# shehryar-malik/icrl

Hardware: AMD Instinct MI355X
Metric: env-steps/sec (ICRL outer loop, HCWithPos-v0) (higher is better)
Workload: dtype f32

## Files before the change

icrl_amd/csrc/ppo_common.h:

```cpp
#pragma once
#include "common.h"

namespace icrl {

typedef float f32x4 __attribute__((ext_vector_type(4)));
typedef unsigned long long u64;
#define MFMA_F32(a, b, c) __builtin_amdgcn_mfma_f32_16x16x4f32((a), (b), (c), 0, 0, 0)

constexpr int RB = 64;
constexpr int HD = 64;
constexpr int SH = 72;
constexpr int MAXB = 256;

struct TrainArgs {
  PolLayout L;
  float* params;
  float* exp_avg;
  float* exp_avg_sq;
  int* adam_t;
  icrl_buffer_t buf;
  const int* perms;
  const float* nu;
  icrl_ppo_hyper_t hp;
  float* stats;
  u64* xch;
  unsigned t_magic;
  const struct PlanStep* plan_steps;
  const struct PlanChunk* plan_chunks;
  int n_steps;
  u64* gx;
};

struct PlanStep {
  float step_size, inv_bc2_sqrt;
  int nb_flags;

  int perm_base;
};
constexpr int NB_MASK = 0x3ff, NB_FIRST = 10, NB_LAST = 11, NB_EPOCH = 12;
struct PlanChunk {
  int perm_base, rows;
};

__device__ __forceinline__ float sum16(float v) { return row_sum(v); }

__device__ __forceinline__ float tile_colsum(const f32x4& t) {
  return quad_rows_sum((t[0] + t[1]) + (t[2] + t[3]));
}

__device__ __forceinline__ unsigned long long stamp() {
  unsigned long long t;
  asm volatile("s_memtime %0\n\ts_waitcnt lgkmcnt(0)" : "=s"(t)::"memory");
  return t;
}
#define STAMP(slot)                                                        \
  if (prof) {                                                              \
    __builtin_amdgcn_sched_barrier(0);                                     \
    const unsigned long long now_ = stamp();                               \
    __builtin_amdgcn_sched_barrier(0);                                     \
    ph[slot] += now_ - t_last;                                             \
    t_last = now_;                                                         \
  }

__device__ __forceinline__ void lds_barrier() { asm volatile("s_waitcnt lgkmcnt(0)\n\ts_barrier" ::: "memory"); }

__device__ __forceinline__ f32x4 lds128(const float* p) { return *reinterpret_cast<const f32x4*>(p); }

__device__ __forceinline__ void acc_put(float& slot, float v) { asm("v_accvgpr_write_b32 %0, %1" : "=a"(slot) : "v"(v)); }
__device__ __forceinline__ void acc_set(float& slot, float v) { asm("v_accvgpr_write_b32 %0, %1" : "+a"(slot) : "v"(v)); }
__device__ __forceinline__ float acc_get(const float& slot) {
  float v;
  asm("v_accvgpr_read_b32 %0, %1" : "=v"(v) : "a"(slot));
  return v;
}

struct Cursor {
  int e, p, m;
};

constexpr int XCD_STRIDE = 8;
__device__ __forceinline__ int xcc_word(int j) { return j < 4 ? 28 + j : 56 + j; }
__device__ __forceinline__ int xcc_word12(int j) { return j < 8 ? 24 + j : 48 + j; }
__device__ __forceinline__ bool run_on_one_xcd(unsigned long long* xch, int j, int M, bool wide = false) {
  const unsigned long long me = 0x100ull | (unsigned long long)xcc_id();
  __hip_atomic_store(xch + (wide ? xcc_word12(j) : xcc_word(j)), me, __ATOMIC_RELAXED, __HIP_MEMORY_SCOPE_AGENT);
  bool same = true;
  for (int o = 0; o < M; ++o) {
    if (o == j) continue;
    unsigned long long v = 0;
    for (int spins = 0; spins < (1 << 18); ++spins) {
      v = __hip_atomic_load(xch + (wide ? xcc_word12(o) : xcc_word(o)), __ATOMIC_RELAXED, __HIP_MEMORY_SCOPE_AGENT);
      if (v != 0) break;
      __builtin_amdgcn_s_sleep(8);
    }
    same = same && v == me;
  }
  return same;
}
__device__ __forceinline__ bool packed_slot(int M, int n_runs, int& run, int& j) {
  const int id = (int)blockIdx.x, per = XCD_STRIDE * M;
  run = (id / per) * XCD_STRIDE + (id & (XCD_STRIDE - 1));
  j = (id % per) / XCD_STRIDE;
  return run < n_runs;
}
inline int packed_grid(int M, int n_runs) {
  static const bool off = getenv("ICRL_NO_XCD_PACK") != nullptr;
  static const int cus_per_xcd = [] {
    int dev = 0, cus = 0;
    if (hipGetDevice(&dev) != hipSuccess || hipDeviceGetAttribute(&cus, hipDeviceAttributeMultiprocessorCount, dev) != hipSuccess || cus < XCD_STRIDE) return 32;
    return cus / XCD_STRIDE;
  }();
  const int groups = (n_runs + XCD_STRIDE - 1) / XCD_STRIDE;
  if (off || groups * M > cus_per_xcd - 2) return 0;
  return n_runs >= XCD_STRIDE ? groups * XCD_STRIDE * M : XCD_STRIDE * (M - 1) + n_runs;
}
template <class K>
inline int launch_update_single(K kernel, int M, dim3 block, size_t dyn_lds, hipStream_t s, TrainArgs& arg) {
  const int pg = packed_grid(M, 1);
  hipError_t e = launch_coresident(kernel, dim3(pg ? pg : M), block, dyn_lds, s, arg, pg ? 1 : 0);
  if (e == hipErrorCooperativeLaunchTooLarge && pg) {
    (void)hipGetLastError();
    e = launch_coresident(kernel, dim3(M), block, dyn_lds, s, arg, 0);
  }
  return (int)e;
}

#if defined(__HIP_DEVICE_COMPILE__) && !defined(__gfx950__) && !defined(__gfx942__)
#error "libicrl_hip: the XCD-local exchange of the persistent kernels is written for gfx950 (CDNA4) / gfx942"
#endif

int launch_train_rows(const TrainArgs& a, int nt1, bool discrete, bool split, hipStream_t s);
int launch_train_pairs(const TrainArgs& a, int nt1, bool discrete, hipStream_t s);
int launch_train_halves(const TrainArgs& a, bool discrete, int parts, hipStream_t s);
int launch_train_halves_batch(const TrainArgs* d_args, int n_runs, int obs, bool discrete, int parts, bool prof, hipStream_t s);
int launch_train_quarters_wide(const TrainArgs& a, bool discrete, hipStream_t s);
int launch_train_quarters_wide2(const TrainArgs& a, bool discrete, hipStream_t s);
constexpr int HALVES_MAX_RUNS = 40;
constexpr int QUARTERS_MAX_RUNS = 16;
int launch_train_rows_batch(const TrainArgs* d_args, int n_runs, int nt1, bool discrete, bool split, hipStream_t s);
int launch_train_pairs_batch(const TrainArgs* d_args, int n_runs, int obs, int nt1, bool discrete, bool prof, hipStream_t s);


}
```

icrl_amd/csrc/ppo_train.hip:

```cpp
#include "ppo_common.h"

namespace icrl {

constexpr int TH = 512;
constexpr int SO = 24;

template <int NT1>
struct Smem {
  static constexpr int O16 = 16 * NT1, SX = O16 + 8;
  static constexpr int W1 = 0;
  static constexpr int W2 = W1 + HD * SX;
  static constexpr int WH = W2 + HD * SH;
  static constexpr int B1 = WH + 16 * SH;
  static constexpr int B2 = B1 + HD;
  static constexpr int BH = B2 + HD;
  static constexpr int LS = BH + 16;
  static constexpr int X = LS + 16;
  static constexpr int H1 = X + RB * SX;
  static constexpr int H2 = H1 + RB * SH;
  static constexpr int DZ = H2 + RB * SH;
  static constexpr int DO = DZ + RB * SH;
  static constexpr int RED1 = DO + RB * SO;
  static constexpr int RED2 = RED1 + 4 * HD;
  static constexpr int PBH = RED2 + 4 * HD;
  static constexpr int PLS = PBH + 64;
  static constexpr int PST = PLS + 64;
  static constexpr int MISC = PST + 32;
  static constexpr int GAU = MISC + 48;
  static constexpr int TOTAL = GAU + 48;
  static constexpr int ACT = DZ, OLP = DZ + 16, ADR = DZ + 17, ADC = DZ + 18;
};

template <int NT1, bool DISC>
__global__ void __launch_bounds__(TH, 2) ppo_train_kernel(TrainArgs a) {
  using S = Smem<NT1>;
  constexpr int SX = S::SX;
  constexpr int NT1H = NT1 / 2;
  constexpr int XR = (SX + 7) / 8;
  static_assert(NT1 >= 2, "obs tiles are split between the two column halves");
  extern __shared__ __attribute__((aligned(16))) float sm[];
  const int role = blockIdx.x;
  const int tid = threadIdx.x;
  const int lane = tid & 63;
  const int w = __builtin_amdgcn_readfirstlane(tid >> 6);
  const int rt = w & 3, hf = w >> 2;
  const int r = lane & 15, q = lane >> 4;
  const PolLayout& L = a.L;
  const int O = L.O, A = L.A;
  const int n_out = role == 0 ? A : 1;
  const int T = a.buf.T, N = a.buf.N;
  const int n_total = T * N;
  const int B = a.hp.batch_size;
  const int n_mb = (n_total + B - 1) / B;
  const int n_epochs = a.hp.n_epochs;
  const float nu = a.nu[0];

  const int gW1 = L.W1[role], gb1 = L.b1[role], gW2 = L.W2[role], gb2 = L.b2[role];
  const int gWh = role == 0 ? L.Wa : (role == 1 ? L.Wv : L.Wc);
  const int gbh = role == 0 ? L.ba : (role == 1 ? L.bv : L.bc);

  for (int i = tid; i < HD * SX; i += TH) { const int j = i / SX, k = i % SX; sm[S::W1 + i] = k < O ? a.params[gW1 + j * O + k] : 0.f; }
  for (int i = tid; i < HD * SH; i += TH) { const int j = i / SH, k = i % SH; sm[S::W2 + i] = k < HD ? a.params[gW2 + j * HD + k] : 0.f; }
  for (int i = tid; i < 16 * SH; i += TH) { const int o = i / SH, k = i % SH; sm[S::WH + i] = (o < n_out && k < HD) ? a.params[gWh + o * HD + k] : 0.f; }
  if (tid < HD) { sm[S::B1 + tid] = a.params[gb1 + tid]; sm[S::B2 + tid] = a.params[gb2 + tid]; }
  if (tid < 16) { sm[S::BH + tid] = tid < n_out ? a.params[gbh + tid] : 0.f; sm[S::LS + tid] = (!DISC && role == 0 && tid < A) ? a.params[L.log_std + tid] : 0.f; }

  f32x4 mW1[NT1H], vW1[NT1H], gW1r[NT1H], mW2[2], vW2[2], gW2r[2], mWh, vWh, gWhr;
#pragma unroll
  for (int c = 0; c < NT1H; ++c)
#pragma unroll
    for (int i = 0; i < 4; ++i) {
      const int j = 16 * rt + 4 * q + i, k = 16 * (hf * NT1H + c) + r;
      mW1[c][i] = k < O ? a.exp_avg[gW1 + j * O + k] : 0.f;
      vW1[c][i] = k < O ? a.exp_avg_sq[gW1 + j * O + k] : 0.f;
    }
#pragma unroll
  for (int c = 0; c < 2; ++c)
#pragma unroll
    for (int i = 0; i < 4; ++i) {
      const int j = 16 * rt + 4 * q + i, k = 16 * (2 * hf + c) + r;
      mW2[c][i] = a.exp_avg[gW2 + j * HD + k];
      vW2[c][i] = a.exp_avg_sq[gW2 + j * HD + k];
    }
#pragma unroll
  for (int i = 0; i < 4; ++i) {
    const int o = 4 * q + i, j = 16 * rt + r;
    const bool own = hf == 0 && o < n_out;
    mWh[i] = own ? a.exp_avg[gWh + o * HD + j] : 0.f;
    vWh[i] = own ? a.exp_avg_sq[gWh + o * HD + j] : 0.f;
  }
  int vec_g = -1, vec_s = 0;
  if (tid < 64) { vec_g = gb1 + tid; vec_s = S::B1 + tid; }
  else if (tid < 128) { vec_g = gb2 + tid - 64; vec_s = S::B2 + tid - 64; }
  else if (tid < 144) { if (tid - 128 < n_out) { vec_g = gbh + tid - 128; vec_s = S::BH + tid - 128; } }
  else if (tid < 160) { if (!DISC && role == 0 && tid - 144 < A) { vec_g = L.log_std + tid - 144; vec_s = S::LS + tid - 144; } }
  float mB = 0.f, vB = 0.f, gB = 0.f;
  if (vec_g >= 0) { mB = a.exp_avg[vec_g]; vB = a.exp_avg_sq[vec_g]; }

  const int t0 = a.adam_t[0];
  double b1pow = pow((double)a.hp.adam_beta1, (double)t0), b2pow = pow((double)a.hp.adam_beta2, (double)t0);
  const float w1 = (float)(1.0 - (double)a.hp.adam_beta1);
  const float w2 = (float)(1.0 - (double)a.hp.adam_beta2);
  const float clip = a.hp.clip_range;
  const float vclip = role == 1 ? a.hp.clip_range_reward_vf : a.hp.clip_range_cost_vf;
  const float vcoef = role == 1 ? a.hp.reward_vf_coef : a.hp.cost_vf_coef;

  auto cur_rows = [&](const Cursor& c) {
    int left = B - c.m;
    if (n_total - c.p < left) left = n_total - c.p;
    return left < RB ? left : RB;
  };
  auto cur_advance = [&](Cursor c) {
    const int rows = cur_rows(c);
    c.p += rows; c.m += rows;
    if (c.p >= n_total) { c.p = 0; c.m = 0; ++c.e; }
    else if (c.m >= B) c.m = 0;
    return c;
  };
  auto to_off = [&](int idx) -> unsigned {
    unsigned env = __umulhi((unsigned)idx, a.t_magic);
    int t = idx - (int)env * T;
    if (t >= T) { t -= T; ++env; }
    if (t >= T) { t -= T; ++env; }
    return (unsigned)t * (unsigned)N + env;
  };
  const int gb_row = tid >> 3, gpart = tid & 7;
  auto load_idx = [&](const Cursor& c) -> int {
    if (c.e >= n_epochs || gb_row >= cur_rows(c)) return -1;
    return a.perms[(size_t)c.e * n_total + c.p + gb_row];
  };
  float px[XR], pact[2], psc0 = 0.f, psc1 = 0.f, psc2 = 0.f;
  auto issue_rows = [&](int idx) {
    const bool valid = idx >= 0;
    const size_t off = valid ? (size_t)to_off(idx) : 0;
    const float* orow = a.buf.observations + off * O;
#pragma unroll
    for (int i = 0; i < XR; ++i) { const int k = gpart + 8 * i; px[i] = (valid && k < O) ? orow[k] : 0.f; }
    if (role == 0) {
      const float* arow = a.buf.actions + off * a.buf.act_store;
#pragma unroll
      for (int i = 0; i < 2; ++i) { const int k = gpart + 8 * i; pact[i] = (valid && k < a.buf.act_store) ? arow[k] : 0.f; }
      if (gpart == 0) {
        psc0 = valid ? a.buf.log_probs[off] : 0.f;
        psc1 = valid ? a.buf.reward_advantages[off] : 0.f;
        psc2 = valid ? a.buf.cost_advantages[off] : 0.f;
      }
    } else if (gpart == 0) {
      const float* rets = role == 1 ? a.buf.reward_returns : a.buf.cost_returns;
      const float* olds = role == 1 ? a.buf.reward_values : a.buf.cost_values;
      psc1 = valid ? rets[off] : 0.f;
      psc0 = valid ? olds[off] : 0.f;
    }
  };
  auto commit_rows = [&]() {
#pragma unroll
    for (int i = 0; i < XR; ++i) { const int k = gpart + 8 * i; if (k < SX) sm[S::X + gb_row * SX + k] = px[i]; }
    if (role == 0) {
#pragma unroll
      for (int i = 0; i < 2; ++i) sm[S::ACT + gb_row * SH + gpart + 8 * i] = pact[i];
      if (gpart == 0) { sm[S::OLP + gb_row * SH] = psc0; sm[S::ADR + gb_row * SH] = psc1; sm[S::ADC + gb_row * SH] = psc2; }
    } else if (gpart == 0) {
      sm[S::OLP + gb_row * SH] = psc0; sm[S::ADR + gb_row * SH] = psc1;
    }
  };
  float sar = 0.f, sac = 0.f;
  auto mb_rows_at = [&](int p) { const int left = n_total - p; return left < B ? left : B; };
  auto stat_idx = [&](int e, int p) -> int {
    if (role != 0 || e >= n_epochs || tid >= mb_rows_at(p)) return -1;
    return a.perms[(size_t)e * n_total + p + tid];
  };
  auto issue_stats = [&](int idx) {
    sar = 0.f; sac = 0.f;
    if (idx >= 0) {
      const unsigned off = to_off(idx);
      sar = a.buf.reward_advantages[off];
      sac = a.buf.cost_advantages[off];
    }
  };
  float mean_r = 0.f, std_r = 1.f, mean_c = 0.f;
  auto compute_stats = [&](int nb) {
    if (role != 0) return;
    const bool in = tid < nb;
    float s_r = wave_sum_fast(in ? sar : 0.f), s_c = wave_sum_fast(in ? sac : 0.f), s_rr = wave_sum_fast(in ? sar * sar : 0.f);
    lds_barrier();
    if (lane == 0) { sm[S::MISC + 16 + w] = s_r; sm[S::MISC + 24 + w] = s_c; sm[S::MISC + 32 + w] = s_rr; }
    lds_barrier();
    s_r = sm[S::MISC + 16] + sm[S::MISC + 17];
    s_c = sm[S::MISC + 24] + sm[S::MISC + 25];
    s_rr = sm[S::MISC + 32] + sm[S::MISC + 33];
    mean_r = s_r / (float)nb;
    mean_c = s_c / (float)nb;
    const float var = fmaxf(s_rr - s_r * mean_r, 0.f) / (float)(nb - 1);
    std_r = sqrtf(var);
  };
  auto refresh_gauss = [&]() {
    if (!DISC && role == 0 && tid >= 144 && tid < 160) {
      const int k = tid - 144;
      const float sd = __expf(sm[S::LS + k]);
      const float iv = __builtin_amdgcn_rcpf(sd * sd);
      sm[S::GAU + k] = k < A ? iv : 0.f;
      sm[S::GAU + 16 + k] = k < A ? 0.5f * iv : 0.f;
      sm[S::GAU + 32 + k] = k < A ? __logf(sd) + LOG_SQRT_2PI_F : 0.f;
    }
  };
  float st_ent = 0.f, st_pg = 0.f, st_vl = 0.f, st_cf = 0.f, last_loss = 0.f;
  int steps_done = 0, early_stop_epoch = n_epochs, status = 0;
  if (tid == 0) { sm[S::MISC + 12] = 0.f; sm[S::MISC + 13] = 0.f; }

  Cursor c_nx2 = cur_advance(Cursor{0, 0, 0});
  int idx_next = load_idx(c_nx2);
  c_nx2 = cur_advance(c_nx2);
  int idx_nx2 = load_idx(c_nx2);
  issue_rows(load_idx(Cursor{0, 0, 0}));
  issue_stats(stat_idx(0, 0));
  refresh_gauss();
  int s_e = 0, s_p = mb_rows_at(0);
  if (s_p >= n_total) { s_p = 0; s_e = 1; }
  int sidx_next = stat_idx(s_e, s_p);
  __syncthreads();
  commit_rows();
  compute_stats(mb_rows_at(0));
  __syncthreads();

  const bool prof = (a.hp._pad & 1) != 0;
  unsigned long long ph[8] = {0, 0, 0, 0, 0, 0, 0, 0};
  unsigned long long t_last = prof ? stamp() : 0ull;

  unsigned step = 0;
  bool stop = false;
  for (int epoch = 0; epoch < n_epochs && !stop; ++epoch) {
    float kl_sum = 0.f;
    for (int mb = 0; mb < n_mb && !stop; ++mb) {
      ++step;
      const int nb = mb_rows_at(mb * B);
      const float c_mean_r = mean_r, c_mean_c = mean_c;
      const float c_istd_r = 1.f / (std_r + 1e-8f);
      const float cpol_nb = 1.f / ((1.f + nu) * (float)nb);
      issue_stats(sidx_next);
      {
        s_p += mb_rows_at(s_p);
        if (s_p >= n_total) { s_p = 0; ++s_e; }
        sidx_next = stat_idx(s_e, s_p);
      }
#pragma unroll
      for (int c = 0; c < NT1H; ++c) gW1r[c] = f32x4{0.f, 0.f, 0.f, 0.f};
#pragma unroll
      for (int c = 0; c < 2; ++c) gW2r[c] = f32x4{0.f, 0.f, 0.f, 0.f};
      gWhr = f32x4{0.f, 0.f, 0.f, 0.f};
      gB = 0.f;
      float mb_s0 = 0.f, mb_s1 = 0.f, mb_s2 = 0.f, mb_s3 = 0.f, mb_s4 = 0.f;

      const int n_chunks = (nb + RB - 1) / RB;
      for (int ch = 0; ch < n_chunks; ++ch) {
        const int nrows = (nb - ch * RB) < RB ? (nb - ch * RB) : RB;
        if (ch > 0) {
          commit_rows();
          lds_barrier();
        }
        f32x4 h1t[2], h2t[2];
        {
          f32x4 av[NT1], bv[2][NT1];
          const float* pa = sm + S::X + (16 * rt + r) * SX + 4 * q;
          const float* pb = sm + S::W1 + (32 * hf + r) * SX + 4 * q;
#pragma unroll
          for (int js = 0; js < NT1; ++js) {
            av[js] = lds128(pa + 16 * js);
#pragma unroll
            for (int c = 0; c < 2; ++c) bv[c][js] = lds128(pb + c * 16 * SX + 16 * js);
          }
          __builtin_amdgcn_sched_barrier(0);
          f32x4 acc[2];
#pragma unroll
          for (int c = 0; c < 2; ++c) acc[c] = f32x4{0.f, 0.f, 0.f, 0.f};
#pragma unroll
          for (int js = 0; js < NT1; ++js)
#pragma unroll
            for (int e = 0; e < 4; ++e)
#pragma unroll
              for (int c = 0; c < 2; ++c) acc[c] = MFMA_F32(av[js][e], bv[c][js][e], acc[c]);
#pragma unroll
          for (int c = 0; c < 2; ++c) {
            const int col = 32 * hf + 16 * c + r;
            const float bias = sm[S::B1 + col];
#pragma unroll
            for (int i = 0; i < 4; ++i) {
              h1t[c][i] = fast_tanh(acc[c][i] + bias);
              sm[S::H1 + (16 * rt + 4 * q + i) * SH + col] = h1t[c][i];
            }
          }
        }
        issue_rows(idx_next);
        idx_next = idx_nx2;
        c_nx2 = cur_advance(c_nx2);
        idx_nx2 = load_idx(c_nx2);
        lds_barrier();
        {
          f32x4 av[4], bv[2][4];
          const float* pa = sm + S::H1 + (16 * rt + r) * SH + 4 * q;
          const float* pb = sm + S::W2 + (32 * hf + r) * SH + 4 * q;
#pragma unroll
          for (int js = 0; js < 4; ++js) {
            av[js] = lds128(pa + 16 * js);
#pragma unroll
            for (int c = 0; c < 2; ++c) bv[c][js] = lds128(pb + c * 16 * SH + 16 * js);
          }
          __builtin_amdgcn_sched_barrier(0);
          f32x4 acc[2];
#pragma unroll
          for (int c = 0; c < 2; ++c) acc[c] = f32x4{0.f, 0.f, 0.f, 0.f};
#pragma unroll
          for (int js = 0; js < 4; ++js)
#pragma unroll
            for (int e = 0; e < 4; ++e)
#pragma unroll
              for (int c = 0; c < 2; ++c) acc[c] = MFMA_F32(av[js][e], bv[c][js][e], acc[c]);
#pragma unroll
          for (int c = 0; c < 2; ++c) {
            const int col = 32 * hf + 16 * c + r;
            const float bias = sm[S::B2 + col];
#pragma unroll
            for (int i = 0; i < 4; ++i) {
              h2t[c][i] = fast_tanh(acc[c][i] + bias);
              sm[S::H2 + (16 * rt + 4 * q + i) * SH + col] = h2t[c][i];
            }
          }
        }
        lds_barrier();
        if (hf == 0) {
          f32x4 av[4], bv[4];
          const float* pa = sm + S::H2 + (16 * rt + r) * SH + 4 * q;
          const float* pb = sm + S::WH + r * SH + 4 * q;
#pragma unroll
          for (int js = 0; js < 4; ++js) { av[js] = lds128(pa + 16 * js); bv[js] = lds128(pb + 16 * js); }
          __builtin_amdgcn_sched_barrier(0);
          f32x4 acc[4];
#pragma unroll
          for (int js = 0; js < 4; ++js) {
            acc[js] = f32x4{0.f, 0.f, 0.f, 0.f};
#pragma unroll
            for (int e = 0; e < 4; ++e) acc[js] = MFMA_F32(av[js][e], bv[js][e], acc[js]);
          }
          const float bias = sm[S::BH + r];
#pragma unroll
          for (int i = 0; i < 4; ++i)
            sm[S::DO + (16 * rt + 4 * q + i) * SO + r] = ((acc[0][i] + acc[1][i]) + (acc[2][i] + acc[3][i])) + bias;
        }
        lds_barrier();
        STAMP(0)
        {
          const int b = 16 * rt + r;
          const bool valid = b < nrows;
          float* dor = sm + S::DO + b * SO;
          if (role == 0 && DISC) {
            float lg[4], pr[4], zmax = -INFINITY;
#pragma unroll
            for (int i = 0; i < 4; ++i) {
              const int k = q + 4 * i;
              lg[i] = k < A ? dor[k] : -INFINITY;
              zmax = fmaxf(zmax, lg[i]);
            }
            zmax = xor16_max(xor32_max(zmax));
            float se = 0.f;
#pragma unroll
            for (int i = 0; i < 4; ++i) se += (q + 4 * i < A) ? expf(lg[i] - zmax) : 0.f;
            se = quad_rows_sum(se);
            const float lse = zmax + logf(se);
            const int act = (int)sm[S::ACT + b * SH];
            float lp = 0.f, ent = 0.f;
#pragma unroll
            for (int i = 0; i < 4; ++i) {
              const int k = q + 4 * i;
              lg[i] = k < A ? lg[i] - lse : 0.f;
              pr[i] = k < A ? expf(lg[i]) : 0.f;
              lp += (k == act) ? lg[i] : 0.f;
              ent -= pr[i] * lg[i];
            }
            lp = quad_rows_sum(lp);
            ent = quad_rows_sum(ent);
            const float old_lp = sm[S::OLP + b * SH];
            const float ratio = __expf(lp - old_lp);
            const float Ar = (sm[S::ADR + b * SH] - c_mean_r) * c_istd_r;
            const float Ac = sm[S::ADC + b * SH] - c_mean_c;
            const float s1 = Ar * ratio;
            const float rc = fminf(fmaxf(ratio, 1.f - clip), 1.f + clip);
            const float s2 = Ar * rc;
            const float gsel = (s1 <= s2) ? Ar : 0.f;
            const float dlp = valid ? cpol_nb * (-gsel + nu * Ac) * ratio : 0.f;
            const float dent = valid ? a.hp.ent_coef / (float)nb : 0.f;
            lds_barrier();
#pragma unroll
            for (int ii = 0; ii < 2; ++ii) {
              const int k = q + 4 * (2 * hf + ii);
              const float pk = hf == 0 ? pr[ii] : pr[2 + ii];
              const float lk = hf == 0 ? lg[ii] : lg[2 + ii];
              const float dk = k < A ? dlp * ((k == act ? 1.f : 0.f) - pk) + dent * (pk * (lk + ent)) : 0.f;
              dor[k] = dk;
              const float colsum = sum16(dk);
              if (r == 0) { sm[S::PBH + rt * 16 + k] = colsum; sm[S::PLS + rt * 16 + k] = 0.f; }
            }
            if (hf == 0) {
              const float v0 = sum16(valid ? fminf(s1, s2) : 0.f);
              const float v1 = sum16(valid ? Ac * ratio : 0.f);
              const float v2 = sum16(valid ? (fabsf(ratio - 1.f) > clip ? 1.f : 0.f) : 0.f);
              const float v3 = sum16(valid ? old_lp - lp : 0.f);
              const float v4 = sum16(valid ? ent : 0.f);
              if (lane == 0) { sm[S::PST + rt * 8 + 0] = v0; sm[S::PST + rt * 8 + 1] = v1; sm[S::PST + rt * 8 + 2] = v2; sm[S::PST + rt * 8 + 3] = v3; sm[S::PST + rt * 8 + 4] = v4; }
            }
          } else if (role == 0) {
            float dd[4], iv[4];
            float lp = 0.f;
#pragma unroll
            for (int i = 0; i < 4; ++i) {
              const int k = q + 4 * i;
              dd[i] = sm[S::ACT + b * SH + k] - dor[k];
              iv[i] = sm[S::GAU + k];
              lp += -(dd[i] * dd[i]) * sm[S::GAU + 16 + k] - sm[S::GAU + 32 + k];
            }
            lp = quad_rows_sum(lp);
            const float old_lp = sm[S::OLP + b * SH];
            const float ratio = __expf(lp - old_lp);
            const float Ar = (sm[S::ADR + b * SH] - c_mean_r) * c_istd_r;
            const float Ac = sm[S::ADC + b * SH] - c_mean_c;
            const float s1 = Ar * ratio;
            const float rc = fminf(fmaxf(ratio, 1.f - clip), 1.f + clip);
            const float s2 = Ar * rc;
            const float gsel = (s1 <= s2) ? Ar : 0.f;
            const float dlp = valid ? cpol_nb * (-gsel + nu * Ac) * ratio : 0.f;
            lds_barrier();
#pragma unroll
            for (int ii = 0; ii < 2; ++ii) {
              const int i = 2 * hf + ii;
              const int k = q + 4 * i;
              const float ddi = hf == 0 ? dd[ii] : dd[2 + ii];
              const float ivi = hf == 0 ? iv[ii] : iv[2 + ii];
              const float dk = dlp * (ddi * ivi);
              const float lk = (k < A) ? dlp * ((ddi * ddi) * ivi - 1.f) : 0.f;
              dor[k] = dk;
              const float colsum = sum16(dk);
              const float lssum = sum16(lk);
              if (r == 0) { sm[S::PBH + rt * 16 + k] = colsum; sm[S::PLS + rt * 16 + k] = lssum; }
            }
            if (hf == 0) {
              const float v0 = sum16(valid ? fminf(s1, s2) : 0.f);
              const float v1 = sum16(valid ? Ac * ratio : 0.f);
              const float v2 = sum16(valid ? (fabsf(ratio - 1.f) > clip ? 1.f : 0.f) : 0.f);
              const float v3 = sum16(valid ? old_lp - lp : 0.f);
              if (lane == 0) { sm[S::PST + rt * 8 + 0] = v0; sm[S::PST + rt * 8 + 1] = v1; sm[S::PST + rt * 8 + 2] = v2; sm[S::PST + rt * 8 + 3] = v3; }
            }
          } else {
            const float v = dor[0];
            const float R = sm[S::ADR + b * SH];
            float vp = v, pass = 1.f;
            if (vclip >= 0.f) {
              const float old = sm[S::OLP + b * SH];
              const float dv = v - old;
              vp = old + fminf(fmaxf(dv, -vclip), vclip);
              pass = (dv >= -vclip && dv <= vclip) ? 1.f : 0.f;
            }
            const float e = vp - R;
            const float d0 = valid ? vcoef * 2.f * e / (float)nb * pass : 0.f;
            lds_barrier();
            if (hf == 0) {
              if (q == 0) {
                dor[0] = d0;
#pragma unroll
                for (int k = 1; k < 16; ++k) dor[k] = 0.f;
              }
              const float colsum = sum16(d0);
              const float se = sum16(valid ? e * e : 0.f);
              if (lane == 0) {
                sm[S::PBH + rt * 16] = colsum;
#pragma unroll
                for (int k = 1; k < 16; ++k) sm[S::PBH + rt * 16 + k] = 0.f;
                sm[S::PST + rt * 8 + 0] = se;
              }
            }
          }
        }
        lds_barrier();
        STAMP(1)
        {
          const f32x4 av = lds128(sm + S::DO + (16 * rt + r) * SO + 4 * q);
          float bv[2][4];
          const float* pb = sm + S::WH + (4 * q) * SH + 32 * hf + r;
#pragma unroll
          for (int e = 0; e < 4; ++e)
#pragma unroll
            for (int c = 0; c < 2; ++c) bv[c][e] = pb[e * SH + 16 * c];
          f32x4 acc[2];
#pragma unroll
          for (int c = 0; c < 2; ++c) acc[c] = f32x4{0.f, 0.f, 0.f, 0.f};
#pragma unroll
          for (int e = 0; e < 4; ++e)
#pragma unroll
            for (int c = 0; c < 2; ++c) acc[c] = MFMA_F32(av[e], bv[c][e], acc[c]);
#pragma unroll
          for (int c = 0; c < 2; ++c) {
            const int col = 32 * hf + 16 * c + r;
#pragma unroll
            for (int i = 0; i < 4; ++i) {
              acc[c][i] = acc[c][i] * (1.f - h2t[c][i] * h2t[c][i]);
              sm[S::DZ + (16 * rt + 4 * q + i) * SH + col] = acc[c][i];
            }
            const float cs = tile_colsum(acc[c]);
            if (q == 0) sm[S::RED2 + rt * HD + col] = cs;
          }
        }
        lds_barrier();
        if (hf == 0) {
          float av[4][4], bv[4][4];
          const float* pa = sm + S::DO + (4 * q) * SO + r;
          const float* pb = sm + S::H2 + (4 * q) * SH + 16 * rt + r;
#pragma unroll
          for (int js = 0; js < 4; ++js)
#pragma unroll
            for (int e = 0; e < 4; ++e) { av[js][e] = pa[(16 * js + e) * SO]; bv[js][e] = pb[(16 * js + e) * SH]; }
          __builtin_amdgcn_sched_barrier(0);
          f32x4 acc[4];
#pragma unroll
          for (int js = 0; js < 4; ++js) {
            acc[js] = f32x4{0.f, 0.f, 0.f, 0.f};
#pragma unroll
            for (int e = 0; e < 4; ++e) acc[js] = MFMA_F32(av[js][e], bv[js][e], acc[js]);
          }
#pragma unroll
          for (int i = 0; i < 4; ++i) gWhr[i] += (acc[0][i] + acc[1][i]) + (acc[2][i] + acc[3][i]);
        }
        if (tid >= 64 && tid < 128) {
          const int j = tid - 64;
          gB += (sm[S::RED2 + j] + sm[S::RED2 + HD + j]) + (sm[S::RED2 + 2 * HD + j] + sm[S::RED2 + 3 * HD + j]);
        } else if (tid >= 128 && tid < 144) {
          const int k = tid - 128;
          gB += (sm[S::PBH + k] + sm[S::PBH + 16 + k]) + (sm[S::PBH + 32 + k] + sm[S::PBH + 48 + k]);
        } else if (tid >= 144 && tid < 160) {
          const int k = tid - 144;
          gB += (sm[S::PLS + k] + sm[S::PLS + 16 + k]) + (sm[S::PLS + 32 + k] + sm[S::PLS + 48 + k]);
        }
        if (tid == 0) {
          mb_s0 += (sm[S::PST + 0] + sm[S::PST + 8]) + (sm[S::PST + 16] + sm[S::PST + 24]);
          mb_s1 += (sm[S::PST + 1] + sm[S::PST + 9]) + (sm[S::PST + 17] + sm[S::PST + 25]);
          mb_s2 += (sm[S::PST + 2] + sm[S::PST + 10]) + (sm[S::PST + 18] + sm[S::PST + 26]);
          mb_s3 += (sm[S::PST + 3] + sm[S::PST + 11]) + (sm[S::PST + 19] + sm[S::PST + 27]);
          if (DISC) mb_s4 += (sm[S::PST + 4] + sm[S::PST + 12]) + (sm[S::PST + 20] + sm[S::PST + 28]);
        }
        lds_barrier();
        {
          f32x4 av[4];
          const float* pa = sm + S::DZ + (16 * rt + r) * SH + 4 * q;
          const float* pb = sm + S::W2 + (4 * q) * SH + 32 * hf + r;
#pragma unroll
          for (int js = 0; js < 4; ++js) av[js] = lds128(pa + 16 * js);
          float bv[4][2][4];
#pragma unroll
          for (int js = 0; js < 4; ++js)
#pragma unroll
            for (int e = 0; e < 4; ++e)
#pragma unroll
              for (int c = 0; c < 2; ++c) bv[js][c][e] = pb[(16 * js + e) * SH + 16 * c];
          __builtin_amdgcn_sched_barrier(0);
          f32x4 acc[2];
#pragma unroll
          for (int c = 0; c < 2; ++c) acc[c] = f32x4{0.f, 0.f, 0.f, 0.f};
#pragma unroll
          for (int js = 0; js < 4; ++js)
#pragma unroll
            for (int e = 0; e < 4; ++e)
#pragma unroll
              for (int c = 0; c < 2; ++c) acc[c] = MFMA_F32(av[js][e], bv[js][c][e], acc[c]);
          float a2[4][4], b2v[4][2][4];
          const float* pa2 = sm + S::DZ + (4 * q) * SH + 16 * rt + r;
          const float* pb2 = sm + S::H1 + (4 * q) * SH + 32 * hf + r;
#pragma unroll
          for (int js = 0; js < 4; ++js)
#pragma unroll
            for (int e = 0; e < 4; ++e) {
              a2[js][e] = pa2[(16 * js + e) * SH];
#pragma unroll
              for (int c = 0; c < 2; ++c) b2v[js][c][e] = pb2[(16 * js + e) * SH + 16 * c];
            }
#pragma unroll
          for (int js = 0; js < 4; ++js)
#pragma unroll
            for (int e = 0; e < 4; ++e)
#pragma unroll
              for (int c = 0; c < 2; ++c) gW2r[c] = MFMA_F32(a2[js][e], b2v[js][c][e], gW2r[c]);
#pragma unroll
          for (int c = 0; c < 2; ++c) {
            const int col = 32 * hf + 16 * c + r;
#pragma unroll
            for (int i = 0; i < 4; ++i) {
              acc[c][i] = acc[c][i] * (1.f - h1t[c][i] * h1t[c][i]);
              sm[S::H2 + (16 * rt + 4 * q + i) * SH + col] = acc[c][i];
            }
            const float cs = tile_colsum(acc[c]);
            if (q == 0) sm[S::RED1 + rt * HD + col] = cs;
          }
        }
        lds_barrier();
        {
          float av[4][4];
          const float* pa = sm + S::H2 + (4 * q) * SH + 16 * rt + r;
          const float* pb = sm + S::X + (4 * q) * SX + 16 * hf * NT1H + r;
#pragma unroll
          for (int js = 0; js < 4; ++js)
#pragma unroll
            for (int e = 0; e < 4; ++e) av[js][e] = pa[(16 * js + e) * SH];
#pragma unroll
          for (int js = 0; js < 4; ++js) {
            float bv[NT1H][4];
#pragma unroll
            for (int e = 0; e < 4; ++e)
#pragma unroll
              for (int c = 0; c < NT1H; ++c) bv[c][e] = pb[(16 * js + e) * SX + 16 * c];
#pragma unroll
            for (int e = 0; e < 4; ++e)
#pragma unroll
              for (int c = 0; c < NT1H; ++c) gW1r[c] = MFMA_F32(av[js][e], bv[c][e], gW1r[c]);
          }
        }
        if (tid < 64) gB += (sm[S::RED1 + tid] + sm[S::RED1 + HD + tid]) + (sm[S::RED1 + 2 * HD + tid] + sm[S::RED1 + 3 * HD + tid]);
        lds_barrier();
        STAMP(2)
      }

      if (!DISC && role == 0 && tid >= 144 && tid < 144 + A) gB += -a.hp.ent_coef;

      float ss = 0.f;
#pragma unroll
      for (int c = 0; c < NT1H; ++c)
#pragma unroll
        for (int i = 0; i < 4; ++i) ss += gW1r[c][i] * gW1r[c][i];
#pragma unroll
      for (int c = 0; c < 2; ++c)
#pragma unroll
        for (int i = 0; i < 4; ++i) ss += gW2r[c][i] * gW2r[c][i];
#pragma unroll
      for (int i = 0; i < 4; ++i) ss += gWhr[i] * gWhr[i];
      if (vec_g >= 0) ss += gB * gB;
      ss = wave_sum_fast(ss);
      if (lane == 0) sm[S::MISC + w] = ss;
      lds_barrier();
      if (tid == 0) {
        ss = ((sm[S::MISC + 0] + sm[S::MISC + 1]) + (sm[S::MISC + 2] + sm[S::MISC + 3])) +
             ((sm[S::MISC + 4] + sm[S::MISC + 5]) + (sm[S::MISC + 6] + sm[S::MISC + 7]));
        bool want_stop = false;
        float mean_kl = 0.f;
        if (role == 0) {
          kl_sum += mb_s3 / (float)nb;
          if (mb == n_mb - 1) {
            mean_kl = kl_sum / (float)n_mb;
            if (a.hp.use_target_kl && mean_kl > 1.5f * a.hp.target_kl) { want_stop = true; early_stop_epoch = epoch; }
          }
        }
        const unsigned tag = step | (want_stop ? 0x80000000u : 0u);
        __hip_atomic_store(a.xch + (step & 1) * 4 + role, ((u64)tag << 32) | (u64)__float_as_uint(ss), __ATOMIC_RELAXED,
                           __HIP_MEMORY_SCOPE_AGENT);
        ++steps_done;
        if (role == 0) {
          float ent = 0.f;
          if (DISC) ent = mb_s4 / (float)nb;
          else for (int k = 0; k < A; ++k) ent += HALF_LOG_2PI_PLUS_HALF_F + sm[S::LS + k];
          const float entropy_loss = -ent;
          const float pl = (-(mb_s0 / (float)nb) + nu * (mb_s1 / (float)nb)) / (1.f + nu);
          st_ent += entropy_loss; st_pg += pl; st_cf += mb_s2 / (float)nb;
          last_loss = pl + a.hp.ent_coef * entropy_loss;
          if (mb == n_mb - 1) { a.stats[32 + epoch] = mean_kl; a.stats[7] = mean_kl; }
        } else {
          const float vl = mb_s0 / (float)nb;
          st_vl += vl;
          last_loss = vl;
        }
      }
      STAMP(3)
      commit_rows();
      {
        const int pn = (mb + 1 < n_mb) ? (mb + 1) * B : 0;
        compute_stats(mb_rows_at(pn));
      }
      STAMP(4)
      if (tid < 3) {
        u64 v = 0;
        int spins = 0;
        bool ok = false;
        while (spins < (1 << 24)) {
          v = __hip_atomic_load(a.xch + (step & 1) * 4 + tid, __ATOMIC_RELAXED, __HIP_MEMORY_SCOPE_AGENT);
          if ((unsigned)((v >> 32) & 0x7fffffffu) == step) { ok = true; break; }
          __builtin_amdgcn_s_sleep(1);
          ++spins;
        }
        sm[S::MISC + 8 + tid] = __uint_as_float((unsigned)(v & 0xffffffffu));
        if (tid == 0) sm[S::MISC + 12] = (v >> 63) ? 1.f : 0.f;
        if (!ok) sm[S::MISC + 13] = 1.f;
      } else if (tid == 3) {
        b1pow *= (double)a.hp.adam_beta1;
        b2pow *= (double)a.hp.adam_beta2;
        sm[S::MISC + 14] = (float)((double)a.hp.lr / (1.0 - b1pow));
        sm[S::MISC + 15] = (float)(1.0 / sqrt(1.0 - b2pow));
      }
      lds_barrier();
      STAMP(5)
      const float total = sqrtf((sm[S::MISC + 8] + sm[S::MISC + 9]) + sm[S::MISC + 10]);
      stop = sm[S::MISC + 12] != 0.f;
      if (sm[S::MISC + 13] != 0.f) { status = 1; stop = true; }
      float coef = a.hp.max_grad_norm / (total + 1e-6f);
      coef = coef > 1.f ? 1.f : coef;

      const float step_size = sm[S::MISC + 14];
      const float inv_bc2_sqrt = sm[S::MISC + 15];
      const float b2f = a.hp.adam_beta2, epsf = a.hp.adam_eps;
      auto adam = [&](float g, float& m, float& v, float p) -> float {
        g = g * coef;
        m = m + (g - m) * w1;
        v = v * b2f + w2 * (g * g);
        const float denom = __builtin_amdgcn_sqrtf(v) * inv_bc2_sqrt + epsf;
        return p - step_size * (m * __builtin_amdgcn_rcpf(denom));
      };
      if (status == 0) {
#pragma unroll
        for (int c = 0; c < NT1H; ++c)
#pragma unroll
          for (int i = 0; i < 4; ++i) {
            const int j = 16 * rt + 4 * q + i, k = 16 * (hf * NT1H + c) + r;
            if (k < O) { float* pw = sm + S::W1 + j * SX + k; float m_ = mW1[c][i], v_ = vW1[c][i]; *pw = adam(gW1r[c][i], m_, v_, *pw); mW1[c][i] = m_; vW1[c][i] = v_; }
          }
#pragma unroll
        for (int c = 0; c < 2; ++c)
#pragma unroll
          for (int i = 0; i < 4; ++i) {
            float* pw = sm + S::W2 + (16 * rt + 4 * q + i) * SH + 16 * (2 * hf + c) + r;
            float m_ = mW2[c][i], v_ = vW2[c][i];
            *pw = adam(gW2r[c][i], m_, v_, *pw);
            mW2[c][i] = m_; vW2[c][i] = v_;
          }
        if (hf == 0) {
#pragma unroll
          for (int i = 0; i < 4; ++i) {
            const int o = 4 * q + i;
            if (o < n_out) { float* pw = sm + S::WH + o * SH + 16 * rt + r; float m_ = mWh[i], v_ = vWh[i]; *pw = adam(gWhr[i], m_, v_, *pw); mWh[i] = m_; vWh[i] = v_; }
          }
        }
        if (vec_g >= 0) sm[vec_s] = adam(gB, mB, vB, sm[vec_s]);
        refresh_gauss();
      }
      if (tid == 0) { sm[S::MISC + 12] = 0.f; sm[S::MISC + 13] = 0.f; }
      lds_barrier();
      STAMP(6)
    }
  }

  __syncthreads();
  for (int i = tid; i < HD * O; i += TH) { const int j = i / O, k = i % O; a.params[gW1 + i] = sm[S::W1 + j * SX + k]; }
  for (int i = tid; i < HD * HD; i += TH) { const int j = i / HD, k = i % HD; a.params[gW2 + i] = sm[S::W2 + j * SH + k]; }
  for (int i = tid; i < n_out * HD; i += TH) { const int o = i / HD, k = i % HD; a.params[gWh + i] = sm[S::WH + o * SH + k]; }
  if (vec_g >= 0) { a.params[vec_g] = sm[vec_s]; a.exp_avg[vec_g] = mB; a.exp_avg_sq[vec_g] = vB; }
#pragma unroll
  for (int c = 0; c < NT1H; ++c)
#pragma unroll
    for (int i = 0; i < 4; ++i) {
      const int j = 16 * rt + 4 * q + i, k = 16 * (hf * NT1H + c) + r;
      if (k < O) { a.exp_avg[gW1 + j * O + k] = mW1[c][i]; a.exp_avg_sq[gW1 + j * O + k] = vW1[c][i]; }
    }
#pragma unroll
  for (int c = 0; c < 2; ++c)
#pragma unroll
    for (int i = 0; i < 4; ++i) {
      const int j = 16 * rt + 4 * q + i, k = 16 * (2 * hf + c) + r;
      a.exp_avg[gW2 + j * HD + k] = mW2[c][i];
      a.exp_avg_sq[gW2 + j * HD + k] = vW2[c][i];
    }
  if (hf == 0) {
#pragma unroll
    for (int i = 0; i < 4; ++i) {
      const int o = 4 * q + i, j = 16 * rt + r;
      if (o < n_out) { a.exp_avg[gWh + o * HD + j] = mWh[i]; a.exp_avg_sq[gWh + o * HD + j] = vWh[i]; }
    }
  }
  if (tid == 0 && prof) {
    for (int k = 0; k < 7; ++k) {
      const int slot = 12 + 7 * role + k;
      if (slot < 32) a.stats[slot] = (float)((double)ph[k] / (double)(steps_done > 0 ? steps_done : 1));
    }
  }
  if (tid == 0) {
    if (role == 0) {
      a.stats[0] = (float)early_stop_epoch;
      a.stats[1] = (float)steps_done;
      a.stats[2] = st_ent; a.stats[3] = st_pg; a.stats[6] = st_cf;
      a.stats[8] = last_loss;
      a.stats[11] = (float)status;
      a.adam_t[0] = t0 + steps_done;
    } else if (role == 1) {
      a.stats[4] = st_vl; a.stats[9] = last_loss;
    } else {
      a.stats[5] = st_vl; a.stats[10] = last_loss;
    }
  }
}

__global__ void ppo_perm_offsets_kernel(const int* __restrict__ perms, long long n, int T, int N, int* __restrict__ out) {
  const long long i = (long long)blockIdx.x * blockDim.x + threadIdx.x;
  if (i >= n) return;
  const int idx = perms[i];
  const int env = idx / T, t = idx - env * T;
  out[i] = t * N + env;
}

__global__ void ppo_plan_kernel(const int* adam_t, int n_steps, int n_mb, int n_total, int B, double lr, double b1, double b2,
                                PlanStep* steps, PlanChunk* chunks, int two_per_step) {
  const int i = blockIdx.x * blockDim.x + threadIdx.x;
  if (i >= n_steps + 2) return;
  if (i >= n_steps) { steps[i] = PlanStep{0.f, 0.f, 0, 0}; return; }
  const int e = i / n_mb, mb = i % n_mb, p = mb * B;
  const int nb = n_total - p < B ? n_total - p : B;
  const int cpm = (B + RB - 1) / RB;
  const int nb_last = n_total - (n_mb - 1) * B;
  const int cpe = (n_mb - 1) * cpm + (nb_last + RB - 1) / RB;
  const int g0 = e * cpe + mb * cpm, nch = (nb + RB - 1) / RB;
  const double t = (double)(adam_t[0] + i + 1);
  steps[i] = PlanStep{(float)(lr / (1.0 - pow(b1, t))), (float)(1.0 / sqrt(1.0 - pow(b2, t))),
                      nb | ((mb == 0) << NB_FIRST) | ((mb == n_mb - 1) << NB_LAST) | (e << NB_EPOCH), e * n_total + p};
  if (chunks == nullptr) return;
  if (two_per_step) {
    for (int c = 0; c < 2; ++c) chunks[2 * i + c] = c < nch ? PlanChunk{e * n_total + p + RB * c, nb - RB * c < RB ? nb - RB * c : RB} : PlanChunk{0, 0};
    if (i == n_steps - 1)
      for (int c = 0; c < 10; ++c) chunks[2 * n_steps + c] = PlanChunk{0, 0};
    return;
  }
  for (int c = 0; c < nch; ++c) chunks[g0 + c] = PlanChunk{e * n_total + p + RB * c, nb - RB * c < RB ? nb - RB * c : RB};
  if (i == n_steps - 1)
    for (int c = 0; c < 5; ++c) chunks[g0 + nch + c] = PlanChunk{0, 0};
}

}

using namespace icrl;

template <int NT1, bool DISC>
static int launch_train(const TrainArgs& a, hipStream_t s) {
  static_assert(Smem<NT1>::TOTAL * sizeof(float) <= 160 * 1024, "LDS budget");
  const size_t bytes = (size_t)Smem<NT1>::TOTAL * sizeof(float);
  hipError_t e = hipFuncSetAttribute((const void*)ppo_train_kernel<NT1, DISC>, hipFuncAttributeMaxDynamicSharedMemorySize, (int)bytes);
  if (e != hipSuccess) return (int)e;
  TrainArgs arg = a;
  return (int)launch_coresident(ppo_train_kernel<NT1, DISC>, dim3(3), dim3(TH), bytes, s, arg);
}

static bool quarters_default() {
  static const int v = [] { const char* e = getenv("ICRL_QUARTERS"); return e != nullptr ? (e[0] == '1' ? 1 : 0) : 1; }();
  return v != 0;
}

static int prepare_train(const icrl_policy_t* pol, float* exp_avg, float* exp_avg_sq, int32_t* adam_step, const icrl_buffer_t* buf,
                         const int32_t* perms, const float* nu, const icrl_ppo_hyper_t* hp, float* stats, void* sync_ws,
                         hipStream_t s, TrainArgs& a, int* err, int n_runs) {
  auto bad = [&](int e) { *err = e; return -1; };
  if (pol->arch != nullptr || pol->h1 != HD || pol->h2 != HD)
    return bad(fail("icrl_ppo_lag_train: hidden widths (%d, %d)%s; the persistent update kernels are built for %d x %d (the reference's default net_arch)", pol->h1, pol->h2,
                    pol->arch != nullptr ? " with an `arch` descriptor" : "", HD, HD));
  if (pol->obs_dim < 1 || pol->obs_dim > 128 || pol->act_dim < 1 || pol->act_dim > 16)
    return bad(fail("icrl_ppo_lag_train: obs_dim %d (1..128) / act_dim %d (1..16)", pol->obs_dim, pol->act_dim));
  if (hp->batch_size < 2 || hp->batch_size > MAXB || hp->n_epochs < 1)
    return bad(fail("icrl_ppo_lag_train: batch_size %d (2..%d: one minibatch = at most four 64-row chunks of one workgroup), n_epochs %d (>= 1)", hp->batch_size, MAXB, hp->n_epochs));
  if (hp->n_epochs >= (1 << 19)) return bad(fail("icrl_ppo_lag_train: n_epochs %d, limit 2^19", hp->n_epochs));
  if (hp->batch_size > 128 && (hp->_pad & 2))
    return bad(fail("icrl_ppo_lag_train: batch_size %d: the column-split tiles kernel (hp->_pad & 2) stops at 128 rows", hp->batch_size));
  if (buf->obs_dim != pol->obs_dim || buf->T < 1)
    return bad(fail("icrl_ppo_lag_train: buffer obs_dim %d vs policy %d, T = %d", buf->obs_dim, pol->obs_dim, buf->T));
  if ((long long)buf->T * buf->N >= (1ll << 31) || (long long)buf->T * buf->N * (pol->obs_dim > 16 ? pol->obs_dim : 16) >= (1ll << 30))
    return bad(fail("icrl_ppo_lag_train: %d x %d transitions x obs_dim %d overflow the kernel's 32-bit element offsets (limit 2^30 floats per plane)", buf->T, buf->N, pol->obs_dim));
  if (pol->discrete && buf->act_store != 1) return bad(fail("icrl_ppo_lag_train: discrete policy needs act_store = 1 (action index), got %d", buf->act_store));
  a.L = make_pol_layout(pol->obs_dim, pol->act_dim, pol->h1, pol->h2, pol->discrete);
  a.params = pol->params; a.exp_avg = exp_avg; a.exp_avg_sq = exp_avg_sq; a.adam_t = adam_step;
  a.buf = *buf; a.perms = perms; a.nu = nu; a.hp = *hp; a.stats = stats; a.xch = (u64*)sync_ws;
  a.t_magic = buf->T == 1 ? 0xFFFFFFFFu : (unsigned)((1ull << 32) / (unsigned long long)buf->T);
  a.plan_steps = nullptr; a.plan_chunks = nullptr; a.n_steps = 0; a.gx = nullptr;
  hipError_t e = hipMemsetAsync(sync_ws, 0, 512, s);
  if (e != hipSuccess) return bad((int)e);
  e = hipMemsetAsync(stats, 0, (32 + hp->n_epochs) * sizeof(float), s);
  if (e != hipSuccess) return bad((int)e);
  const int nt1 = (pol->obs_dim + 15) / 16;
  if (nt1 > 8 || (hp->_pad & 2)) {
    if (hp->batch_size > 128) return bad(fail("icrl_ppo_lag_train: batch_size %d with obs_dim %d: the column-split tiles kernel stops at 128 rows", hp->batch_size, pol->obs_dim));
    return 3;
  }
  const int n_total = buf->T * buf->N;
  const int n_mb = (n_total + hp->batch_size - 1) / hp->batch_size;
  const long long n_steps = (long long)hp->n_epochs * n_mb;
  if (n_steps >= (1ll << 21)) return bad(fail("icrl_ppo_lag_train: %lld optimiser steps per call, limit 2^21", n_steps));
  PlanStep* steps = reinterpret_cast<PlanStep*>((char*)sync_ws + 512);
  PlanChunk* chunks = reinterpret_cast<PlanChunk*>(steps + n_steps + 2);
  a.plan_steps = steps; a.plan_chunks = chunks; a.n_steps = (int)n_steps;
  {
    int* offs = reinterpret_cast<int*>((char*)sync_ws + ICRL_PPO_PLAN_BYTES(n_steps));
    const long long n = (long long)hp->n_epochs * n_total;
    hipLaunchKernelGGL(ppo_perm_offsets_kernel, dim3((unsigned)((n + 255) / 256)), dim3(256), 0, s, perms, n, buf->T, buf->N, offs);
    a.perms = offs;
  }
  const bool quarters_wide = nt1 > 4 && n_runs == 1 && !(hp->_pad & (4 | 32)) && quarters_default();
  static const bool one_pass = [] { const char* e = getenv("ICRL_QUARTERS_PASSES"); return e == nullptr || e[0] != '1'; }();
  const bool quarters_wide2 = quarters_wide && one_pass && hp->batch_size > RB && hp->batch_size <= 2 * RB;
  const bool rows = !quarters_wide && ((hp->_pad & 4) || nt1 > 4);
  const bool split = rows && hp->batch_size > RB && hp->batch_size <= 2 * RB && !(hp->_pad & 8);
  const bool halves = !rows && n_runs <= HALVES_MAX_RUNS && nt1 <= 2 && !(hp->_pad & 16);
  const bool quarters = halves && n_runs <= QUARTERS_MAX_RUNS && !(hp->_pad & 32) && quarters_default();
  hipLaunchKernelGGL(ppo_plan_kernel, dim3((unsigned)((n_steps + 2 + 255) / 256)), dim3(256), 0, s, adam_step, (int)n_steps, n_mb,
                     n_total, hp->batch_size, (double)hp->lr, (double)hp->adam_beta1, (double)hp->adam_beta2, steps, chunks, (int)(split || quarters_wide2));
  if (split || halves || quarters_wide) {
    const size_t off = (ICRL_PPO_PLAN_BYTES(n_steps) + 4 * (size_t)hp->n_epochs * n_total + 255) / 256 * 256;
    a.gx = reinterpret_cast<u64*>((char*)sync_ws + off);
    e = hipMemsetAsync(a.gx, 0, ICRL_PPO_SPLIT_BYTES, s);
    if (e != hipSuccess) return bad((int)e);
  }
  if (quarters_wide) return quarters_wide2 ? 7 : 6;
  return rows ? (split ? 2 : 1) : (halves ? (quarters ? 5 : 4) : 0);
}

static int train_generic(const icrl_policy_t* pol, float* exp_avg, float* exp_avg_sq, int32_t* adam_step, const icrl_buffer_t* buf,
                         const int32_t* perms, const float* nu, const icrl_ppo_hyper_t* hp, float* stats, void* sync_ws, hipStream_t s) {
  if (hp->batch_size < 2 || hp->n_epochs < 1) return fail("icrl_ppo_lag_train: batch_size %d (>= 2), n_epochs %d (>= 1)", hp->batch_size, hp->n_epochs);
  if (pol->arch != nullptr) { if (int e = policy_generic_check(pol, "icrl_ppo_lag_train")) return e; }
  else if (pol->h1 != pol->h2 || pol->h1 % 64 != 0 || pol->h1 > 256 || pol->obs_dim < 1 || pol->obs_dim > 1024 || pol->act_dim < 1 || pol->act_dim > 16)
    return fail("icrl_ppo_lag_train: hidden widths (%d, %d), obs_dim %d, act_dim %d: the persistent kernels are built for %d x %d (narrower layers stored "
                "zero-padded), obs <= 128, act <= 16; the generic-shape path for a common padded width that is a multiple of 64 up to 256, obs <= 1024",
                pol->h1, pol->h2, pol->obs_dim, pol->act_dim, HD, HD);
  if (buf->obs_dim != pol->obs_dim || buf->T < 1) return fail("icrl_ppo_lag_train: buffer obs_dim %d vs policy %d, T = %d", buf->obs_dim, pol->obs_dim, buf->T);
  if ((long long)buf->T * buf->N * (pol->obs_dim > 16 ? pol->obs_dim : 16) >= (1ll << 31))
    return fail("icrl_ppo_lag_train: %d x %d transitions x obs_dim %d overflow 32-bit element offsets", buf->T, buf->N, pol->obs_dim);
  if (pol->discrete && buf->act_store != 1) return fail("icrl_ppo_lag_train: discrete policy needs act_store = 1 (action index), got %d", buf->act_store);
  const int n_total = buf->T * buf->N;
  const int n_mb = (n_total + hp->batch_size - 1) / hp->batch_size;
  const long long n_steps = (long long)hp->n_epochs * n_mb;
  hipError_t e = hipMemsetAsync(stats, 0, (32 + hp->n_epochs) * sizeof(float), s);
  if (e != hipSuccess) return (int)e;
  int* offs = reinterpret_cast<int*>((char*)sync_ws + ICRL_PPO_PLAN_BYTES(n_steps));
  const long long n = (long long)hp->n_epochs * n_total;
  hipLaunchKernelGGL(ppo_perm_offsets_kernel, dim3((unsigned)((n + 255) / 256)), dim3(256), 0, s, perms, n, buf->T, buf->N, offs);
  char* scratch = (char*)sync_ws + ICRL_PPO_SYNC_BYTES(hp->n_epochs, n_mb, n_total);
  const int err = launch_train_generic(pol, exp_avg, exp_avg_sq, adam_step, buf, offs, nu, hp, stats, scratch, sync_ws, s);
  if (err == 0 && !policy_is_wide(pol)) return icrl_policy_prepare(pol, (void*)s);
  return err;
}

extern "C" int icrl_ppo_generic_row_floats(const icrl_policy_t* pol) { return generic_row_floats(pol); }

extern "C" int icrl_ppo_lag_train(const icrl_policy_t* pol, float* exp_avg, float* exp_avg_sq, int32_t* adam_step,
                                  const icrl_buffer_t* buf, const int32_t* perms, const float* nu,
                                  const icrl_ppo_hyper_t* hp, float* stats, void* sync_ws, void* stream) {
  TrainArgs a;
  hipStream_t s = (hipStream_t)stream;
  if (policy_is_wide(pol) || hp->batch_size > MAXB)
    return train_generic(pol, exp_avg, exp_avg_sq, adam_step, buf, perms, nu, hp, stats, sync_ws, s);
  int err = 0;
  const int kind = prepare_train(pol, exp_avg, exp_avg_sq, adam_step, buf, perms, nu, hp, stats, sync_ws, s, a, &err, 1);
  if (kind < 0) return err;
  const int nt1 = (pol->obs_dim + 15) / 16;
  if (kind == 4 || kind == 5) return launch_train_halves(a, pol->discrete != 0, kind == 5 ? 4 : 2, s);
  if (kind == 6) return launch_train_quarters_wide(a, pol->discrete != 0, s);
  if (kind == 7) return launch_train_quarters_wide2(a, pol->discrete != 0, s);
  if (kind == 0) return launch_train_pairs(a, nt1, pol->discrete != 0, s);
  if (kind <= 2) return launch_train_rows(a, nt1, pol->discrete != 0, kind == 2, s);
  if (pol->discrete) {
    if (nt1 <= 2) return launch_train<2, true>(a, s);
    if (nt1 <= 4) return launch_train<4, true>(a, s);
    return launch_train<8, true>(a, s);
  }
  if (nt1 <= 2) return launch_train<2, false>(a, s);
  if (nt1 <= 4) return launch_train<4, false>(a, s);
  return launch_train<8, false>(a, s);
}

extern "C" int icrl_ppo_lag_train_batch(int n_runs, const icrl_ppo_train_job_t* jobs, void* args_ws, long long args_ws_bytes,
                                        void* stream) {
  if (n_runs < 1 || n_runs > 65535) return fail("icrl_ppo_lag_train_batch: n_runs = %d (1..65535)", n_runs);
  if (args_ws == nullptr || args_ws_bytes < (long long)n_runs * (long long)sizeof(TrainArgs))
    return fail("icrl_ppo_lag_train_batch: args_ws holds %lld B, %d runs need %lld (ICRL_BATCH_ARGS_BYTES each)", args_ws_bytes, n_runs,
                (long long)n_runs * (long long)sizeof(TrainArgs));
  static_assert(sizeof(TrainArgs) <= ICRL_BATCH_ARGS_BYTES, "ICRL_BATCH_ARGS_BYTES");
  hipStream_t s = (hipStream_t)stream;
  TrainArgs* d_args = (TrainArgs*)args_ws;
  int kind0 = -1;
  const icrl_ppo_train_job_t& j0 = jobs[0];
  for (int r = 0; r < n_runs; ++r) {
    const icrl_ppo_train_job_t& j = jobs[r];
    if (j.pol->obs_dim != j0.pol->obs_dim || j.pol->act_dim != j0.pol->act_dim || j.pol->discrete != j0.pol->discrete ||
        j.hp->batch_size != j0.hp->batch_size || j.hp->n_epochs != j0.hp->n_epochs || j.hp->_pad != j0.hp->_pad ||
        j.buf->T != j0.buf->T || j.buf->N != j0.buf->N || j.buf->act_store != j0.buf->act_store)
      return fail("icrl_ppo_lag_train_batch: run %d differs from run 0 in a shape (obs / act / discrete / batch_size / n_epochs / T / N): the runs of a batch share one grid", r);
    TrainArgs a;
    int err = 0;
    const int kind = prepare_train(j.pol, j.exp_avg, j.exp_avg_sq, j.adam_step, j.buf, j.perms, j.nu, j.hp, j.stats, j.sync_ws, s, a, &err, n_runs);
    if (kind < 0) return err;
    if (kind == 3) return fail("icrl_ppo_lag_train_batch: the column-split tiles kernel (hp->_pad & 2) has no batched form");
    if (r == 0) kind0 = kind;
    if (kind == 6) return launch_train_quarters_wide(a, j.pol->discrete != 0, s);
    if (kind == 7) return launch_train_quarters_wide2(a, j.pol->discrete != 0, s);
    const int e = put_args(a, d_args + r, s);
    if (e != 0) return e;
  }
  const int nt1 = (j0.pol->obs_dim + 15) / 16;
  if (kind0 == 4 || kind0 == 5) return launch_train_halves_batch(d_args, n_runs, j0.pol->obs_dim, j0.pol->discrete != 0, kind0 == 5 ? 4 : 2, (j0.hp->_pad & 1) != 0, s);
  if (kind0 == 0) return launch_train_pairs_batch(d_args, n_runs, j0.pol->obs_dim, nt1, j0.pol->discrete != 0, (j0.hp->_pad & 1) != 0, s);
  return launch_train_rows_batch(d_args, n_runs, nt1, j0.pol->discrete != 0, kind0 == 2, s);
}
```

icrl_amd/csrc/ppo_train_halves.hip:

```cpp
#include <type_traits>

#include "ppo_common.h"

#ifndef ICRL_HALVES_EARLY_PUBLISH
#define ICRL_HALVES_EARLY_PUBLISH 0
#endif
#ifndef ICRL_HALVES_STAGE_IN_HOP
#define ICRL_HALVES_STAGE_IN_HOP 0
#endif
#ifndef ICRL_HALVES_EARLY_POLL
#define ICRL_HALVES_EARLY_POLL 1
#endif
#ifndef ICRL_HALVES_ADAM_TRIM
#define ICRL_HALVES_ADAM_TRIM 0
#endif
#ifndef ICRL_HALVES_ADAM_PRE
#define ICRL_HALVES_ADAM_PRE 0
#endif
#ifndef ICRL_HALVES_LOSS_WAVES
#define ICRL_HALVES_LOSS_WAVES 4
#endif
#ifndef ICRL_HALVES_POLL_ROLL
#define ICRL_HALVES_POLL_ROLL 0
#endif
#ifndef ICRL_HALVES_OWNER_ADAM
#define ICRL_HALVES_OWNER_ADAM 0
#endif
#ifndef ICRL_HALVES_FLAGS_TOGETHER
#define ICRL_HALVES_FLAGS_TOGETHER 1
#endif
#ifndef ICRL_HALVES_PARTNER_SUM
#define ICRL_HALVES_PARTNER_SUM 1
#endif
#ifndef ICRL_HALVES_FENCES
#define ICRL_HALVES_FENCES 1
#endif
#define HFENCE() do { if (ICRL_HALVES_FENCES) __builtin_amdgcn_sched_barrier(0); } while (0)
#ifndef ICRL_HALVES_LOSS_PRELOAD
#define ICRL_HALVES_LOSS_PRELOAD 1
#endif
#ifndef ICRL_HALVES_ADAM_PRELOAD
#define ICRL_HALVES_ADAM_PRELOAD 0
#endif
#ifndef ICRL_HALVES_LATE_PREFETCH
#define ICRL_HALVES_LATE_PREFETCH 0
#endif
#ifndef ICRL_HALVES_PREFETCH_AT_ADAM
#define ICRL_HALVES_PREFETCH_AT_ADAM 0
#endif
#ifndef ICRL_HALVES_ROLE_SPEC
#define ICRL_HALVES_ROLE_SPEC 0
#endif
#ifndef ICRL_HALVES_IMAGES_FIRST
#define ICRL_HALVES_IMAGES_FIRST 0
#endif
#ifndef ICRL_HALVES_STAGE_IDLE
#define ICRL_HALVES_STAGE_IDLE 0
#endif
#ifndef ICRL_HALVES_SOFFSET
#define ICRL_HALVES_SOFFSET 0
#endif
#ifndef ICRL_HALVES_DEFER_STATS
#define ICRL_HALVES_DEFER_STATS 0
#endif
#ifndef ICRL_HALVES_QUAD_BARRIER
#define ICRL_HALVES_QUAD_BARRIER 1
#endif
#ifndef ICRL_HALVES_POLL_WAVE
#define ICRL_HALVES_POLL_WAVE 4
#endif
#ifndef ICRL_HALVES_FIRST_LOOK
#define ICRL_HALVES_FIRST_LOOK 0
#endif
#ifndef ICRL_HALVES_NORM_LOOK_EARLY
#define ICRL_HALVES_NORM_LOOK_EARLY 0
#endif
#ifndef ICRL_HALVES_QUAD_SPREAD
#define ICRL_HALVES_QUAD_SPREAD 0
#endif

namespace icrl {

constexpr int THH = 512;
constexpr int HR = 32;
constexpr int STH = 40;
constexpr int SRM = 72;
constexpr int SAH = 24;
constexpr int HX_GROUPS = 7;
constexpr int HX_FLAG = HX_GROUPS * THH * 16;
constexpr int HX_BLK = HX_FLAG + 8 * 64;
constexpr int H3_FLAG = 5 * THH * 16;
constexpr int H3_BLK = H3_FLAG + 8 * 64;
constexpr int H3_BASE = 24 * HX_BLK;
static_assert(H3_BASE + 24 * H3_BLK + 3 * 512 <= (int)ICRL_PPO_SPLIT_BYTES, "the exchange of up to four row parts per network lives in the split workspace");

template <int NT1>
struct SmemH {
  static constexpr int O16 = 16 * NT1, SX = O16 + 8;
#if ICRL_HALVES_IMAGES_FIRST
  static constexpr int XT0 = 0;
  static constexpr int XT1 = XT0 + O16 * STH;
  static constexpr int H1T = XT1 + O16 * STH;
  static constexpr int H2T = H1T + HD * STH;
  static constexpr int DZ1T = H2T + HD * STH;
  static constexpr int DZ2T = DZ1T + HD * STH;
  static constexpr int DOT = DZ2T + HD * STH;
  static constexpr int H1R = DOT + 16 * STH;
  static constexpr int DZ2R = H1R + HR * SRM;
  static constexpr int ACT = DZ2R + HR * SRM;
  static constexpr int OLP = ACT + HR * SAH;
  static constexpr int ADR = OLP + HR;
  static constexpr int ADC = ADR + HR;
  static constexpr int PST = ADC + HR;
  static constexpr int PLS = PST + 16;
  static constexpr int MISC = PLS + 32;
  static constexpr int GAU = MISC + 64;
  static constexpr int B1 = GAU + 48;
  static constexpr int B2 = B1 + HD;
  static constexpr int BH = B2 + HD;
  static constexpr int LS = BH + 16;
  static constexpr int HPX = LS + 16;
  static constexpr int DOX = HPX + 2048;
  static constexpr int WH = DOX + 512;
  static constexpr int WHT = WH + 16 * SH;
  static constexpr int W1 = WHT + HD * SAH;
  static constexpr int W2 = W1 + HD * SX;
  static constexpr int W2T = W2 + HD * SH;
  static constexpr int TOTAL = W2T + HD * SH;
#else
  static constexpr int W1 = 0;
  static constexpr int W2 = W1 + HD * SX;
  static constexpr int W2T = W2 + HD * SH;
  static constexpr int WH = W2T + HD * SH;
  static constexpr int WHT = WH + 16 * SH;
  static constexpr int B1 = WHT + HD * SAH;
  static constexpr int B2 = B1 + HD;
  static constexpr int BH = B2 + HD;
  static constexpr int LS = BH + 16;
  static constexpr int GAU = LS + 16;
  static constexpr int XT0 = GAU + 48;
  static constexpr int XT1 = XT0 + O16 * STH;
  static constexpr int H1T = XT1 + O16 * STH;
  static constexpr int H2T = H1T + HD * STH;
  static constexpr int DZ1T = H2T + HD * STH;
  static constexpr int DZ2T = DZ1T + HD * STH;
  static constexpr int DOT = DZ2T + HD * STH;
  static constexpr int H1R = DOT + 16 * STH;
  static constexpr int DZ2R = H1R + HR * SRM;
  static constexpr int HPX = DZ2R + HR * SRM;
  static constexpr int ACT = HPX + 2048;
  static constexpr int OLP = ACT + HR * SAH;
  static constexpr int ADR = OLP + HR;
  static constexpr int ADC = ADR + HR;
  static constexpr int PST = ADC + HR;
  static constexpr int PLS = PST + 16;
  static constexpr int MISC = PLS + 32;
  static constexpr int DOX = MISC + 64;
  static constexpr int TOTAL = DOX + 512;
#endif
};

#define KARGS() ([&]() { const TrainArgs* k_ = ka; asm volatile("" : "+s"(k_)); return k_; }())

template <int NT1>
__device__ __forceinline__ float* halves_smem() {
  __shared__ __attribute__((aligned(16))) float sm[SmemH<NT1>::TOTAL];
  return sm;
}

template <int NT1, bool DISC, int OBS, bool BATCH, int NQ, int ROLE_T = -1, bool PROF = false>
__device__ __forceinline__ void ppo_train_halves_body(const TrainArgs& a, const TrainArgs* const ka, const int slot_j) {
#define GPH(x) (BATCH ? as_global(x) : (x))
  using S = SmemH<NT1>;
  constexpr int SX = S::SX;
  static_assert(NT1 == 2, "one observation tile per weight-gradient wave half");
  float* const sm = halves_smem<NT1>();
  static_assert(NQ == 2 || NQ == 4, "two or four row parts per network");
  constexpr int HRQ = RB / NQ;
  constexpr int NJS = HRQ / 16;
  if ((a.hp._pad & 64) && slot_j == 3 * NQ - 1) return;
  const int role = ROLE_T >= 0 ? ROLE_T : slot_j % 3;
  const int half = slot_j / 3;
  const int tid = threadIdx.x;
  const int lane = tid & 63;
  const int w = __builtin_amdgcn_readfirstlane(tid >> 6);
  constexpr bool SPREAD = NQ == 4 || ICRL_HALVES_QUAD_SPREAD;
  const int rt2 = SPREAD ? w >> 2 : w & 1, fq = SPREAD ? w & 3 : w >> 1;
  const int qp0 = SPREAD ? w ^ 1 : w ^ 2, qp1 = SPREAD ? w ^ 2 : w ^ 4, qp2 = SPREAD ? w ^ 3 : w ^ 6;
  const bool fwd_wave = rt2 < NJS;
  constexpr bool OWNER = NQ == 4 && ICRL_HALVES_OWNER_ADAM;
  const bool owner = !OWNER || (w >> 1) == half;
  constexpr bool STAGE_HOP = ICRL_HALVES_STAGE_IN_HOP || NQ == 4;
  const int jt = w & 3, kh = w >> 2;
  const int r = lane & 15, q = lane >> 4;
  const int O = a.L.O, A = a.L.A;
  const int n_out = role == 0 ? A : 1;
  auto out_of = [&](int i) { return 4 * i + q; };
  auto pos_of = [](int o) { return 4 * (o & 3) + (o >> 2); };
  const int ro = pos_of(r);
  const int T = a.buf.T, N = a.buf.N;
  const float nu = GPH(a.nu)[0];
  const int n_steps = a.n_steps;
  const PlanStep* __restrict__ const plan_steps = GPH(a.plan_steps);
  const PlanChunk* __restrict__ const plan_chunks = GPH(a.plan_chunks);
  const int* __restrict__ const perms = GPH(a.perms);
  const float* const p_s0 = GPH(role == 0 ? a.buf.log_probs : (role == 1 ? a.buf.reward_values : a.buf.cost_values));
  const float* const p_s1 = GPH(role == 0 ? a.buf.reward_advantages : (role == 1 ? a.buf.reward_returns : a.buf.cost_returns));
  const float* const p_s2 = GPH(a.buf.cost_advantages);
  const float* const p_obs = GPH(a.buf.observations);
  const float* const p_act = GPH(a.buf.actions);
  const int AS = a.buf.act_store;

  f32x4 mW1, vW1, gW1r, mW2[2], vW2[2], gW2r[2], mWh, vWh, gWhr;
  const int jb = 16 * jt + r;
  float mb1 = 0.f, vb1 = 0.f, mb2 = 0.f, vb2 = 0.f, mex = 0.f, vex = 0.f, gb1r = 0.f, gb2r = 0.f, gex = 0.f;
  int ex_g = -1, ex_s = S::MISC + 63;
  const bool lowk = kh == 0;
  constexpr int W_BH = 0, W_LS = 1;
  auto w1_addr = [&](int i) { return S::W1 + (16 * jt + 4 * q + i) * SX + 16 * kh + r; };
  auto w2_addr = [&](int cc, int i) { return S::W2 + (16 * jt + 4 * q + i) * SH + 16 * (2 * kh + cc) + r; };
  auto store_w1 = [&](const f32x4& v) {
#pragma unroll
    for (int i = 0; i < 4; ++i) sm[w1_addr(i)] = v[i];
  };
  auto load_own_w1 = [&]() -> f32x4 {
    f32x4 v;
#pragma unroll
    for (int i = 0; i < 4; ++i) v[i] = sm[w1_addr(i)];
    return v;
  };
  auto store_w2 = [&](int cc, const f32x4& v) {
#pragma unroll
    for (int i = 0; i < 4; ++i) sm[w2_addr(cc, i)] = v[i];
    *reinterpret_cast<f32x4*>(sm + S::W2T + (16 * (2 * kh + cc) + r) * SH + 16 * jt + 4 * q) = v;
  };
  auto load_own_w2 = [&](int cc) -> f32x4 { return lds128(sm + S::W2T + (16 * (2 * kh + cc) + r) * SH + 16 * jt + 4 * q); };
  auto store_wh = [&](const f32x4& v) {
#pragma unroll
    for (int i = 0; i < 4; ++i) sm[S::WH + (4 * q + i) * SH + 16 * jt + r] = v[i];
    *reinterpret_cast<f32x4*>(sm + S::WHT + (16 * jt + r) * SAH + 4 * q) = v;
  };
  auto load_own_wh = [&]() -> f32x4 { return lds128(sm + S::WHT + (16 * jt + r) * SAH + 4 * q); };
  for (int i = tid; i < S::TOTAL; i += THH) sm[i] = 0.f;
  __syncthreads();
  {
    const PolLayout& L = a.L;
    const int gW1 = L.W1[role], gb1 = L.b1[role], gW2 = L.W2[role], gb2 = L.b2[role];
    const int gWh = role == 0 ? L.Wa : (role == 1 ? L.Wv : L.Wc);
    const int gbh = role == 0 ? L.ba : (role == 1 ? L.bv : L.bc);
    {
      f32x4 pv;
#pragma unroll
      for (int i = 0; i < 4; ++i) {
        const int j = 16 * jt + 4 * q + i, k = 16 * kh + r;
        const bool mine = k < O;
        pv[i] = mine ? a.params[gW1 + j * O + k] : 0.f;
        mW1[i] = mine ? a.exp_avg[gW1 + j * O + k] : 0.f;
        vW1[i] = mine ? a.exp_avg_sq[gW1 + j * O + k] : 0.f;
      }
      store_w1(pv);
    }
#pragma unroll
    for (int cc = 0; cc < 2; ++cc) {
      f32x4 pv;
#pragma unroll
      for (int i = 0; i < 4; ++i) {
        const int j = 16 * jt + 4 * q + i, k = 16 * (2 * kh + cc) + r;
        pv[i] = a.params[gW2 + j * HD + k];
        mW2[cc][i] = a.exp_avg[gW2 + j * HD + k];
        vW2[cc][i] = a.exp_avg_sq[gW2 + j * HD + k];
      }
      store_w2(cc, pv);
    }
    mWh = vWh = gWhr = f32x4{0.f, 0.f, 0.f, 0.f};
    if (lowk) {
      f32x4 pv;
#pragma unroll
      for (int i = 0; i < 4; ++i) {
        const int o = out_of(i), j = 16 * jt + r;
        pv[i] = o < n_out ? a.params[gWh + o * HD + j] : 0.f;
        mWh[i] = o < n_out ? a.exp_avg[gWh + o * HD + j] : 0.f;
        vWh[i] = o < n_out ? a.exp_avg_sq[gWh + o * HD + j] : 0.f;
      }
      store_wh(pv);
      if (w == W_BH && ro < n_out) { ex_g = gbh + ro; ex_s = S::BH + r; }
      if (w == W_LS && !DISC && role == 0 && ro < A) { ex_g = L.log_std + ro; ex_s = S::LS + r; }
      if (ex_g >= 0) { mex = a.exp_avg[ex_g]; vex = a.exp_avg_sq[ex_g]; }
      if (q == 0) sm[ex_s] = ex_g >= 0 ? a.params[ex_g] : 0.f;
      mb1 = a.exp_avg[gb1 + jb]; vb1 = a.exp_avg_sq[gb1 + jb];
      mb2 = a.exp_avg[gb2 + jb]; vb2 = a.exp_avg_sq[gb2 + jb];
      if (q == 0) { sm[S::B1 + jb] = a.params[gb1 + jb]; sm[S::B2 + jb] = a.params[gb2 + jb]; }
    }
  }

  const int t0 = a.adam_t[0];
  const float w1 = (float)(1.0 - (double)a.hp.adam_beta1);
  const float w2 = (float)(1.0 - (double)a.hp.adam_beta2);
  const float clip = a.hp.clip_range;
  const float vclip = role == 1 ? a.hp.clip_range_reward_vf : a.hp.clip_range_cost_vf;
  const float vcoef = role == 1 ? a.hp.reward_vf_coef : a.hp.cost_vf_coef;
  const float ent_coef = a.hp.ent_coef;
  const float max_grad_norm = a.hp.max_grad_norm, adam_epsf = a.hp.adam_eps, adam_b2f = a.hp.adam_beta2;
  u64* const xch0 = GPH(a.xch);
  u64* const gxp = GPH(a.gx);
  u64* const nx = (half == 0 || OWNER) ? xch0 : reinterpret_cast<u64*>(reinterpret_cast<char*>(gxp) + ICRL_PPO_SPLIT_BYTES - 512 * half);

  constexpr bool STAGE_IDLE = ICRL_HALVES_STAGE_IDLE && NQ == 4;
  const int gb_row = STAGE_IDLE ? (tid >> 4) & 15 : tid >> 4, gpart = tid & 15;
  const int gpos = HRQ * half + (gb_row < HRQ ? gb_row : 0);
  const bool stager = STAGE_IDLE ? tid >= 256 : gb_row < HRQ;
  const bool stager_wave = !STAGE_IDLE || w >= 4;
  constexpr int SW0 = 1;
  const int stid = tid - 64 * SW0;
  auto ld_step = [&](int i) -> int4 {
    asm volatile("" : "+v"(i));
    return *reinterpret_cast<const int4*>(plan_steps + i);
  };
  auto ld_chunk = [&](int g) -> int2 {
    asm volatile("" : "+v"(g));
    return *reinterpret_cast<const int2*>(plan_chunks + g);
  };
  auto chunk_idx = [&](const int2& c) -> int { return perms[c.x + (gpos < c.y ? gpos : 0)]; };
  auto stat_idx = [&](const int4& p) -> int {
    const int nbp = p.z & NB_MASK;
    return perms[p.w + ((stid >= 0 && stid < nbp) ? stid : 0)];
  };
  constexpr int XRL = OBS > 0 ? (OBS + 15) / 16 : NT1;
  float px[XRL], pact = 0.f, psc = 0.f;
  const float* const p_sc = gpart == 0 ? p_s0 : (gpart == 1 ? p_s1 : p_s2);
  const int sc_dst = gpart == 0 ? S::OLP + gb_row : (gpart == 1 ? S::ADR + gb_row : (gpart == 2 ? S::ADC + gb_row : S::MISC + 62));
  auto issue_rows = [&](int idx) {
    const unsigned off = idx >= 0 ? (unsigned)idx : 0u;
    const unsigned ob = off * (unsigned)O;
#pragma unroll
    for (int i = 0; i < XRL; ++i) { const int k = gpart + 16 * i; px[i] = p_obs[ob + (unsigned)(k < O ? k : O - 1)]; }
    pact = p_act[off * (unsigned)AS + (unsigned)(gpart < AS ? gpart : AS - 1)];
    psc = p_sc[off];
  };
  auto commit_rows = [&](int xbase) {
    if (NQ == 4 && !stager) return;
#pragma unroll
    for (int i = 0; i < XRL; ++i) { const int k = gpart + 16 * i; if (OBS > 0 ? k < OBS : k < S::O16) sm[xbase + k * STH + gb_row] = px[i]; }
    if (role == 0) sm[S::ACT + gb_row * SAH + pos_of(gpart)] = gpart < AS ? pact : 0.f;
    sm[sc_dst] = psc;
  };
  float sar = 0.f, sac = 0.f;
  auto issue_stats = [&](int idx) {
    const unsigned off = idx >= 0 ? (unsigned)idx : 0u;
    sar = p_s1[off];
    sac = p_s2[off];
  };
  const bool big_mb = a.hp.batch_size > 128;
  auto stats_partials = [&](int nb) {
    if (role != 0 || w < SW0 || w > SW0 + (big_mb ? 3 : 1)) return;
    const bool in = stid < nb;
    const float s_r = wave_sum_fast(in ? sar : 0.f), s_c = wave_sum_fast(in ? sac : 0.f), s_rr = wave_sum_fast(in ? sar * sar : 0.f);
    if (lane == 0) { sm[S::MISC + 3 * (w - SW0)] = s_r; sm[S::MISC + 3 * (w - SW0) + 1] = s_c; sm[S::MISC + 3 * (w - SW0) + 2] = s_rr; }
  };
  float mean_r = 0.f, istd_r = 1.f, mean_c = 0.f;
  auto read_stats = [&](int nb) {
    if (role != 0) return;
    float s_r = sm[S::MISC + 0] + sm[S::MISC + 3];
    float s_c = sm[S::MISC + 1] + sm[S::MISC + 4];
    float s_rr = sm[S::MISC + 2] + sm[S::MISC + 5];
    if (big_mb) {
      s_r += sm[S::MISC + 6] + sm[S::MISC + 9];
      s_c += sm[S::MISC + 7] + sm[S::MISC + 10];
      s_rr += sm[S::MISC + 8] + sm[S::MISC + 11];
    }
    const float inv = __builtin_amdgcn_rcpf((float)nb);
    mean_r = s_r * inv;
    mean_c = s_c * inv;
    const float var = fmaxf(s_rr - s_r * mean_r, 0.f) * __builtin_amdgcn_rcpf((float)(nb - 1));
    istd_r = __builtin_amdgcn_rcpf(__builtin_amdgcn_sqrtf(var) + 1e-8f);
  };
  auto refresh_gauss = [&]() {
    if (!DISC && role == 0 && w == W_LS && q == 0) {
      const float wex = sm[S::LS + r];
      const float sd = __expf(wex);
      const float iv = __builtin_amdgcn_rcpf(sd * sd);
      sm[S::GAU + r] = ro < A ? iv : 0.f;
      sm[S::GAU + 16 + r] = ro < A ? 0.5f * iv : 0.f;
      sm[S::GAU + 32 + r] = ro < A ? wex + LOG_SQRT_2PI_F : 0.f;
      const float ent = row_sum(ro < A ? HALF_LOG_2PI_PLUS_HALF_F + wex : 0.f);
      if (r == 0) sm[S::MISC + 22] = ent;
    }
  };
  int* const pflag = reinterpret_cast<int*>(sm + S::MISC + 48);
  int pphase = 0;
  constexpr bool QBAR = ICRL_HALVES_QUAD_BARRIER && NQ == 4 && ICRL_HALVES_LOSS_WAVES >= 4;
  auto quad_signal = [&]() {
    if (QBAR) return;
    ++pphase;
    asm volatile("s_waitcnt lgkmcnt(0)" ::: "memory");
    if (lane == 0) __hip_atomic_store(pflag + w, pphase, __ATOMIC_RELAXED, __HIP_MEMORY_SCOPE_WORKGROUP);
  };
  auto quad_wait = [&]() {
    if (QBAR) { lds_barrier(); return; }
    while (true) {
      const int f0 = __hip_atomic_load(pflag + qp0, __ATOMIC_RELAXED, __HIP_MEMORY_SCOPE_WORKGROUP);
      const int f1 = __hip_atomic_load(pflag + qp1, __ATOMIC_RELAXED, __HIP_MEMORY_SCOPE_WORKGROUP);
      const int f2 = __hip_atomic_load(pflag + qp2, __ATOMIC_RELAXED, __HIP_MEMORY_SCOPE_WORKGROUP);
      const int f = f0 < f1 ? (f0 < f2 ? f0 : f2) : (f1 < f2 ? f1 : f2);
      if (f >= pphase) break;
      __builtin_amdgcn_s_sleep(0);
    }
    asm volatile("" ::: "memory");
  };
  const bool book = tid == 64 * 7;
  float* const acc_ent = sm + S::MISC + 56; float* const acc_pg = sm + S::MISC + 57; float* const acc_cf = sm + S::MISC + 58;
  float* const acc_vl = sm + S::MISC + 59; float* const acc_last = sm + S::MISC + 60; float* const acc_kl = sm + S::MISC + 61;
  auto lds_add = [](float* p, float x) { __hip_atomic_fetch_add(p, x, __ATOMIC_RELAXED, __HIP_MEMORY_SCOPE_WORKGROUP); };
  int steps_done = 0, early_stop_epoch = a.hp.n_epochs, status = 0;

  int g_chunk = 0;
  int idx_next = chunk_idx(ld_chunk(1)), idx_nx2 = chunk_idx(ld_chunk(2));
  int2 pc_nx3 = ld_chunk(3);
  issue_rows(chunk_idx(ld_chunk(0)));
  int4 ps_next = ld_step(0), ps_nx2 = ld_step(1), ps_nx3 = ld_step(2);
  issue_stats(stat_idx(ps_next));
  int sidx_next = stat_idx(ps_nx2);
  if (tid == 0) sm[S::MISC + 14] = run_on_one_xcd(xch0, slot_j, 3 * NQ, NQ == 4) ? 1.f : 0.f;
  __syncthreads();
#ifdef ICRL_ASSUME_XCD_LOCAL
  constexpr bool xcd_local = true;
#else
  const bool xcd_local = __builtin_amdgcn_readfirstlane(__float_as_int(sm[S::MISC + 14])) != 0;
#endif
  refresh_gauss();
  int xcur = S::XT0;
  commit_rows(xcur);
  stats_partials(__builtin_amdgcn_readfirstlane(ps_next.z) & NB_MASK);
  __syncthreads();
  read_stats(__builtin_amdgcn_readfirstlane(ps_next.z) & NB_MASK);
  const float inv_n_mb = 1.f / (float)((T * N + a.hp.batch_size - 1) / a.hp.batch_size);
  const bool deep_pf = ICRL_HALVES_PREFETCH_AT_ADAM && a.hp.batch_size <= RB;
  if (deep_pf) {
    const int idx_now = idx_next;
    idx_next = idx_nx2;
    idx_nx2 = chunk_idx(pc_nx3);
    pc_nx3 = ld_chunk(4);
    issue_rows(idx_now);
  }

  const int b = 16 * rt2 + r;
  float* const pt = sm + (4 * q) * STH + b;
  constexpr int JT = OBS / 16;
  constexpr bool TAILQ = OBS > 0 && OBS % 16 >= 1 && OBS % 16 <= 4 && JT < NT1;

  typedef unsigned int raw_u4 __attribute__((ext_vector_type(4)));
  const __amdgpu_buffer_rsrc_t grs = __builtin_amdgcn_make_buffer_rsrc(gxp, 0, (int)ICRL_PPO_SPLIT_BYTES, 0x00020000);
  auto raw_store = [&](int byte_off, const f32x4& v) {
    const raw_u4 u = __builtin_bit_cast(raw_u4, v);
    if (xcd_local) __builtin_amdgcn_raw_buffer_store_b128(u, grs, byte_off, 0, 1);
    else __builtin_amdgcn_raw_buffer_store_b128(u, grs, byte_off, 0, 16);
  };
  auto raw_load = [&](int byte_off) -> f32x4 { return __builtin_bit_cast(f32x4, __builtin_amdgcn_raw_buffer_load_b128(grs, byte_off, 0, 16)); };
  const int lane_slot = tid * 16;
  auto raw_store_u = [&](int uni_off, const f32x4& v) {
    if (!ICRL_HALVES_SOFFSET) { raw_store(uni_off + lane_slot, v); return; }
    const raw_u4 u = __builtin_bit_cast(raw_u4, v);
    if (xcd_local) __builtin_amdgcn_raw_buffer_store_b128(u, grs, lane_slot, uni_off, 1);
    else __builtin_amdgcn_raw_buffer_store_b128(u, grs, lane_slot, uni_off, 16);
  };
  auto raw_load_u = [&](int uni_off) -> f32x4 {
    if (!ICRL_HALVES_SOFFSET) return raw_load(uni_off + lane_slot);
    return __builtin_bit_cast(f32x4, __builtin_amdgcn_raw_buffer_load_b128(grs, lane_slot, uni_off, 16));
  };

  constexpr bool prof = PROF;
  unsigned long long ph[8] = {0, 0, 0, 0, 0, 0, 0, 0};
  unsigned long long t_last = prof ? stamp() : 0ull;

  bool stop = false;
  for (int st = 0; st < n_steps && !stop; ++st) {
    const unsigned step = (unsigned)st + 1u;
    PlanStep ps;
    ps.step_size = __int_as_float(__builtin_amdgcn_readfirstlane(ps_next.x));
    ps.inv_bc2_sqrt = __int_as_float(__builtin_amdgcn_readfirstlane(ps_next.y));
    ps.nb_flags = __builtin_amdgcn_readfirstlane(ps_next.z);
    ps.perm_base = 0;
    ps_next = ps_nx2; ps_nx2 = ps_nx3;
    ps_nx3 = ld_step(st + 3 < n_steps + 2 ? st + 3 : n_steps + 1);
    const int nb = ps.nb_flags & NB_MASK;
    const float inv_nb = __builtin_amdgcn_rcpf((float)nb);
    const float c_mean_r = mean_r, c_mean_c = mean_c, c_istd_r = istd_r;
    const float cpol_nb = inv_nb * __builtin_amdgcn_rcpf(1.f + nu);
    issue_stats(sidx_next);
    sidx_next = stat_idx(ps_nx2);
    float mb_s0 = 0.f, mb_s1 = 0.f, mb_s2 = 0.f, mb_s3 = 0.f, mb_s4 = 0.f;
    const int xrole = ((int)(step & 1) * 3 + role) * NQ * HX_BLK;
    const int xmine = xrole + half * HX_BLK, xtheirs = xrole + (1 - half) * HX_BLK;

    const int n_chunks = (nb + RB - 1) / RB;
    for (int ch = 0; ch < n_chunks; ++ch, ++g_chunk) {
      const int nrows = (nb - ch * RB) < RB ? (nb - ch * RB) : RB;
      if (ch > 0) {
        xcur = xcur == S::XT0 ? S::XT1 : S::XT0;
        commit_rows(xcur);
        lds_barrier();
      }
      const bool valid = HRQ * half + b < nrows;
      f32x4 h1c = f32x4{0.f, 0.f, 0.f, 0.f}, h2c = h1c, outc = h1c;
      if (fwd_wave) {
        float bx[NT1][4];
        const float* pb = sm + xcur + (4 * q) * STH + b;
#pragma unroll
        for (int js = 0; js < NT1; ++js)
#pragma unroll
          for (int e = 0; e < 4; ++e) bx[js][e] = ((OBS == 0 || 16 * js + e < OBS) && !(TAILQ && js == JT)) ? pb[(16 * js + e) * STH] : 0.f;
        const float bt = TAILQ ? sm[xcur + (16 * JT + q) * STH + b] : 0.f;
        const float* pa = sm + S::W1 + (16 * fq + r) * SX + 4 * q;
        f32x4 aw[NT1];
#pragma unroll
        for (int js = 0; js < NT1; ++js)
          if (!(TAILQ && js >= JT)) aw[js] = lds128(pa + 16 * js);
        const float at = TAILQ ? sm[S::W1 + (16 * fq + r) * SX + 16 * JT + q] : 0.f;
        f32x4 z = lds128(sm + S::B1 + 16 * fq + 4 * q);
        HFENCE();
#pragma unroll
        for (int js = 0; js < NT1; ++js)
#pragma unroll
          for (int e = 0; e < 4; ++e)
            if ((OBS == 0 || 16 * js + e < OBS) && !(TAILQ && js >= JT)) z = MFMA_F32(aw[js][e], bx[js][e], z);
        if (TAILQ) z = MFMA_F32(at, bt, z);
#pragma unroll
        for (int i = 0; i < 4; ++i) h1c[i] = fast_tanh(z[i]);
#pragma unroll
        for (int i = 0; i < 4; ++i) pt[S::H1T + (16 * fq + i) * STH] = h1c[i];
        *reinterpret_cast<f32x4*>(sm + S::H1R + b * SRM + 16 * fq + 4 * q) = h1c;
      }
      auto prefetch_next = [&]() {
        const int idx_now = idx_next;
        idx_next = idx_nx2;
        idx_nx2 = chunk_idx(pc_nx3);
        pc_nx3 = ld_chunk(g_chunk + 4);
        issue_rows(idx_now);
      };
      const bool pf_here = !deep_pf;
      if (pf_here && stager_wave && (!ICRL_HALVES_LATE_PREFETCH || !fwd_wave)) prefetch_next();
      f32x4 dout = f32x4{0.f, 0.f, 0.f, 0.f};
      float pl_olp = 0.f, pl_adr = 0.f, pl_adc = 0.f;
      f32x4 pl_act = dout, pl_iv = dout, pl_hiv = dout, pl_lsd = dout, pl_wht = dout;
      if (fwd_wave) {
      quad_signal();
      {
        const float* pa = sm + S::W2 + (16 * fq + r) * SH + 4 * q;
        const f32x4 awo = lds128(pa + 16 * fq);
        f32x4 awp[3];
#pragma unroll
        for (int d = 1; d < 4; ++d) awp[d - 1] = lds128(pa + 16 * ((fq + d) & 3));
        f32x4 z = lds128(sm + S::B2 + 16 * fq + 4 * q);
        if (ICRL_HALVES_LATE_PREFETCH && pf_here) { HFENCE(); prefetch_next(); HFENCE(); }
#pragma unroll
        for (int e = 0; e < 4; ++e) z = MFMA_F32(awo[e], h1c[e], z);
        quad_wait();
        f32x4 hp[3];
        const float* ph1 = sm + S::H1R + b * SRM + 4 * q;
#pragma unroll
        for (int d = 1; d < 4; ++d) hp[d - 1] = lds128(ph1 + 16 * ((fq + d) & 3));
        HFENCE();
#pragma unroll
        for (int d = 0; d < 3; ++d)
#pragma unroll
          for (int e = 0; e < 4; ++e) z = MFMA_F32(awp[d][e], hp[d][e], z);
#pragma unroll
        for (int i = 0; i < 4; ++i) h2c[i] = fast_tanh(z[i]);
#pragma unroll
        for (int i = 0; i < 4; ++i) pt[S::H2T + (16 * fq + i) * STH] = h2c[i];
      }
      {
        const f32x4 aw = lds128(sm + S::WH + r * SH + 16 * fq + 4 * q);
        f32x4 acc = fq == 0 ? lds128(sm + S::BH + 4 * q) : f32x4{0.f, 0.f, 0.f, 0.f};
#pragma unroll
        for (int e = 0; e < 4; ++e) acc = MFMA_F32(aw[e], h2c[e], acc);
        float* const hpx = sm + S::HPX + (rt2 * 4 * 64 + lane) * 4;
        *reinterpret_cast<f32x4*>(hpx + fq * 256) = acc;
        if (ICRL_HALVES_LOSS_PRELOAD) {
          pl_olp = sm[S::OLP + b]; pl_adr = sm[S::ADR + b]; pl_adc = sm[S::ADC + b];
          if (role == 0 && !DISC) {
            pl_act = lds128(sm + S::ACT + b * SAH + 4 * q);
            pl_iv = lds128(sm + S::GAU + 4 * q); pl_hiv = lds128(sm + S::GAU + 16 + 4 * q); pl_lsd = lds128(sm + S::GAU + 32 + 4 * q);
          }
          pl_wht = lds128(sm + S::WHT + (16 * fq + r) * SAH + 4 * q);
        }
        quad_signal(); quad_wait();
        const f32x4 p0 = lds128(hpx), p1 = lds128(hpx + 256), p2 = lds128(hpx + 512), p3 = lds128(hpx + 768);
#pragma unroll
        for (int i = 0; i < 4; ++i) outc[i] = (p0[i] + p1[i]) + (p2[i] + p3[i]);
      }
      STAMP(0)
      float v0 = 0.f, v1 = 0.f, v2 = 0.f, v3 = 0.f, v4 = 0.f;
      f32x4 dls_p = f32x4{0.f, 0.f, 0.f, 0.f};
      constexpr bool DEFER = ICRL_HALVES_DEFER_STATS && ICRL_HALVES_LOSS_WAVES >= 4;
      if (ICRL_HALVES_LOSS_WAVES >= 4 || fq < ICRL_HALVES_LOSS_WAVES) {
        if (role == 0) {
          const int ngp = (A + 3) >> 2;
          float lp = 0.f, ent = 0.f;
          f32x4 g1 = f32x4{0.f, 0.f, 0.f, 0.f}, g2 = f32x4{0.f, 0.f, 0.f, 0.f};
          if (DISC) {
            float lg[4], zmax = -INFINITY;
#pragma unroll
            for (int i = 0; i < 4; ++i) { lg[i] = (out_of(i) < A) ? outc[i] : -INFINITY; zmax = fmaxf(zmax, lg[i]); }
            zmax = xor16_max(xor32_max(zmax));
            float se = 0.f;
#pragma unroll
            for (int i = 0; i < 4; ++i) se += (out_of(i) < A) ? expf(lg[i] - zmax) : 0.f;
            se = quad_rows_sum(se);
            const float lse = zmax + logf(se);
            const int act = (int)sm[S::ACT + b * SAH];
            float pr[4];
#pragma unroll
            for (int i = 0; i < 4; ++i) {
              const int k = out_of(i);
              lg[i] = k < A ? lg[i] - lse : 0.f;
              pr[i] = k < A ? expf(lg[i]) : 0.f;
              lp += (k == act) ? lg[i] : 0.f;
              ent -= pr[i] * lg[i];
            }
            lp = quad_rows_sum(lp);
            ent = quad_rows_sum(ent);
#pragma unroll
            for (int i = 0; i < 4; ++i) {
              const int k = out_of(i);
              g1[i] = k < A ? ((k == act ? 1.f : 0.f) - pr[i]) : 0.f;
              g2[i] = k < A ? pr[i] * (lg[i] + ent) : 0.f;
            }
          } else {
            const f32x4 actv = ICRL_HALVES_LOSS_PRELOAD ? pl_act : lds128(sm + S::ACT + b * SAH + 4 * q);
            const f32x4 iv = ICRL_HALVES_LOSS_PRELOAD ? pl_iv : lds128(sm + S::GAU + 4 * q), hiv = ICRL_HALVES_LOSS_PRELOAD ? pl_hiv : lds128(sm + S::GAU + 16 + 4 * q),
                        lsd = ICRL_HALVES_LOSS_PRELOAD ? pl_lsd : lds128(sm + S::GAU + 32 + 4 * q);
            auto elem = [&](int i) {
              const float dd = actv[i] - outc[i];
              lp += -(dd * dd) * hiv[i] - lsd[i];
              g1[i] = dd * iv[i];
              g2[i] = (out_of(i) < A) ? (dd * dd) * iv[i] - 1.f : 0.f;
            };
            elem(0);
            if (ngp > 1) { elem(1); if (ngp > 2) { elem(2); elem(3); } }
            lp = quad_rows_sum(lp);
          }
          const float old_lp = ICRL_HALVES_LOSS_PRELOAD ? pl_olp : sm[S::OLP + b];
          const float ratio = __expf(lp - old_lp);
          const float Ar = ((ICRL_HALVES_LOSS_PRELOAD ? pl_adr : sm[S::ADR + b]) - c_mean_r) * c_istd_r;
          const float Ac = (ICRL_HALVES_LOSS_PRELOAD ? pl_adc : sm[S::ADC + b]) - c_mean_c;
          const float s1 = Ar * ratio;
          const float rc = fminf(fmaxf(ratio, 1.f - clip), 1.f + clip);
          const float s2 = Ar * rc;
          const float gsel = (s1 <= s2) ? Ar : 0.f;
          const float dlp = valid ? cpol_nb * (-gsel + nu * Ac) * ratio : 0.f;
          if (DISC) {
            const float dent = valid ? ent_coef * inv_nb : 0.f;
#pragma unroll
            for (int i = 0; i < 4; ++i) dout[i] = dlp * g1[i] + dent * g2[i];
          } else {
            f32x4 t = f32x4{0.f, 0.f, 0.f, 0.f};
            auto dls = [&](int i) { dout[i] = dlp * g1[i]; if (DEFER) dls_p[i] = dlp * g2[i]; else t[i] = row_sum(dlp * g2[i]); };
            dls(0);
            if (ngp > 1) { dls(1); if (ngp > 2) { dls(2); dls(3); } }
            if (!DEFER && fq == 0 && r == 0) *reinterpret_cast<f32x4*>(sm + S::PLS + 16 * rt2 + 4 * q) = t;
          }
          const bool cnt = valid && q == 0;
          v0 = cnt ? fminf(s1, s2) : 0.f; v1 = cnt ? Ac * ratio : 0.f; v2 = (cnt && fabsf(ratio - 1.f) > clip) ? 1.f : 0.f;
          v3 = cnt ? old_lp - lp : 0.f; v4 = cnt ? ent : 0.f;
        } else {
          const float v = quad_rows_sum(q == 0 ? outc[0] : 0.f);
          const float R = ICRL_HALVES_LOSS_PRELOAD ? pl_adr : sm[S::ADR + b];
          float vp = v, pass = 1.f;
          if (vclip >= 0.f) {
            const float old = ICRL_HALVES_LOSS_PRELOAD ? pl_olp : sm[S::OLP + b];
            const float dv = v - old;
            vp = old + fminf(fmaxf(dv, -vclip), vclip);
            pass = (dv >= -vclip && dv <= vclip) ? 1.f : 0.f;
          }
          const float e = vp - R;
          const float d0 = valid ? vcoef * 2.f * e * inv_nb * pass : 0.f;
          dout[0] = q == 0 ? d0 : 0.f;
          v0 = (valid && q == 0) ? e * e : 0.f;
        }
        if (!DEFER && fq == 0) {
          v0 = row_sum(v0); v1 = row_sum(v1); v2 = row_sum(v2); v3 = row_sum(v3);
          if (DISC) v4 = row_sum(v4);
          if (lane == 0) { float* pst = sm + S::PST + 8 * rt2; pst[0] = v0; pst[1] = v1; pst[2] = v2; pst[3] = v3; pst[4] = v4; }
        }
      }
#if ICRL_HALVES_LOSS_WAVES < 4
      {
        float* const dox = sm + S::DOX + (rt2 * 64 + lane) * 4;
        if (fq == 0) *reinterpret_cast<f32x4*>(dox) = dout;
        quad_signal();
        if (fq >= ICRL_HALVES_LOSS_WAVES) { quad_wait(); dout = lds128(dox); }
      }
#endif
      STAMP(1)
      f32x4 dz2c, dz1c;
      {
        const int ng = (n_out + 3) >> 2;
        const f32x4 aw = ICRL_HALVES_LOSS_PRELOAD ? pl_wht : lds128(sm + S::WHT + (16 * fq + r) * SAH + 4 * q);
        f32x4 acc = MFMA_F32(aw[0], dout[0], (f32x4{0.f, 0.f, 0.f, 0.f}));
        if (ng > 1) {
          acc = MFMA_F32(aw[1], dout[1], acc);
          if (ng > 2) { acc = MFMA_F32(aw[2], dout[2], acc); acc = MFMA_F32(aw[3], dout[3], acc); }
        }
#pragma unroll
        for (int i = 0; i < 4; ++i) dz2c[i] = fmaf(-(h2c[i] * h2c[i]), acc[i], acc[i]);
#pragma unroll
        for (int i = 0; i < 4; ++i) pt[S::DZ2T + (16 * fq + i) * STH] = dz2c[i];
        *reinterpret_cast<f32x4*>(sm + S::DZ2R + b * SRM + 16 * fq + 4 * q) = dz2c;
        if (fq == 0) {
#pragma unroll
          for (int i = 0; i < 4; ++i) pt[S::DOT + i * STH] = dout[i];
        }
      }
      quad_signal();
      if (DEFER && fq == 0) {
        if (role == 0 && !DISC) {
          f32x4 t;
#pragma unroll
          for (int i = 0; i < 4; ++i) t[i] = row_sum(dls_p[i]);
          if (r == 0) *reinterpret_cast<f32x4*>(sm + S::PLS + 16 * rt2 + 4 * q) = t;
        }
        v0 = row_sum(v0); v1 = row_sum(v1); v2 = row_sum(v2); v3 = row_sum(v3);
        if (DISC) v4 = row_sum(v4);
        if (lane == 0) { float* pst = sm + S::PST + 8 * rt2; pst[0] = v0; pst[1] = v1; pst[2] = v2; pst[3] = v3; pst[4] = v4; }
      }
      {
        const float* pa = sm + S::W2T + (16 * fq + r) * SH + 4 * q;
        const f32x4 awo = lds128(pa + 16 * fq);
        f32x4 awp[3];
#pragma unroll
        for (int d = 1; d < 4; ++d) awp[d - 1] = lds128(pa + 16 * ((fq + d) & 3));
        f32x4 acc = f32x4{0.f, 0.f, 0.f, 0.f};
#pragma unroll
        for (int e = 0; e < 4; ++e) acc = MFMA_F32(awo[e], dz2c[e], acc);
        quad_wait();
        f32x4 dp[3];
        const float* pz = sm + S::DZ2R + b * SRM + 4 * q;
#pragma unroll
        for (int d = 1; d < 4; ++d) dp[d - 1] = lds128(pz + 16 * ((fq + d) & 3));
        HFENCE();
#pragma unroll
        for (int d = 0; d < 3; ++d)
#pragma unroll
          for (int e = 0; e < 4; ++e) acc = MFMA_F32(awp[d][e], dp[d][e], acc);
#pragma unroll
        for (int i = 0; i < 4; ++i) dz1c[i] = fmaf(-(h1c[i] * h1c[i]), acc[i], acc[i]);
      }
#pragma unroll
      for (int i = 0; i < 4; ++i) pt[S::DZ1T + (16 * fq + i) * STH] = dz1c[i];
      } else if (QBAR) {
        lds_barrier(); lds_barrier(); lds_barrier();
      }
      STAMP(2)
      if (ch == 0) {
        gW1r = gW2r[0] = gW2r[1] = gWhr = f32x4{0.f, 0.f, 0.f, 0.f};
        gb1r = 0.f; gb2r = 0.f; gex = 0.f;
      }
      lds_barrier();
      const bool last_chunk = ch + 1 == n_chunks;
      {
        f32x4 az[2] = {f32x4{0.f, 0.f, 0.f, 0.f}, f32x4{0.f, 0.f, 0.f, 0.f}};
        const float* pa = sm + S::DZ2T + (16 * jt + r) * STH + 4 * q;
#pragma unroll
        for (int js = 0; js < NJS; ++js) az[js] = lds128(pa + 16 * js);
        f32x4 bh[2][2];
#pragma unroll
        for (int cc = 0; cc < 2; ++cc) {
          const float* pb = sm + S::H1T + (16 * (2 * kh + cc) + r) * STH + 4 * q;
#pragma unroll
          for (int js = 0; js < NJS; ++js) bh[cc][js] = lds128(pb + 16 * js);
        }
        HFENCE();
#pragma unroll
        for (int cc = 0; cc < 2; ++cc) {
#pragma unroll
          for (int js = 0; js < NJS; ++js)
#pragma unroll
            for (int e = 0; e < 4; ++e) gW2r[cc] = MFMA_F32(az[js][e], bh[cc][js][e], gW2r[cc]);
        }
        if (lowk) {
          const float s = ((az[0][0] + az[0][1]) + (az[0][2] + az[0][3])) + ((az[1][0] + az[1][1]) + (az[1][2] + az[1][3]));
          gb2r += quad_rows_sum(s);
        }
      }
      {
        f32x4 az[2] = {f32x4{0.f, 0.f, 0.f, 0.f}, f32x4{0.f, 0.f, 0.f, 0.f}};
        const float* pa = sm + S::DZ1T + (16 * jt + r) * STH + 4 * q;
#pragma unroll
        for (int js = 0; js < NJS; ++js) az[js] = lds128(pa + 16 * js);
        const float* pb = sm + xcur + (16 * kh + r) * STH + 4 * q;
        f32x4 bx[2];
#pragma unroll
        for (int js = 0; js < NJS; ++js) bx[js] = lds128(pb + 16 * js);
        HFENCE();
#pragma unroll
        for (int js = 0; js < NJS; ++js)
#pragma unroll
          for (int e = 0; e < 4; ++e) gW1r = MFMA_F32(az[js][e], bx[js][e], gW1r);
        if (last_chunk && 16 * kh + r >= O) gW1r = f32x4{0.f, 0.f, 0.f, 0.f};
        if (lowk) {
          const float s = ((az[0][0] + az[0][1]) + (az[0][2] + az[0][3])) + ((az[1][0] + az[1][1]) + (az[1][2] + az[1][3]));
          gb1r += quad_rows_sum(s);
        }
      }
      if (ICRL_HALVES_EARLY_PUBLISH && last_chunk) {
        raw_store_u(xmine + 1 * THH * 16, gW2r[0]);
        raw_store_u(xmine + 2 * THH * 16, gW2r[1]);
      }
      if (lowk) {
        f32x4 ao[2] = {f32x4{0.f, 0.f, 0.f, 0.f}, f32x4{0.f, 0.f, 0.f, 0.f}}, bh[2];
        const float* pa = sm + S::DOT + r * STH + 4 * q;
        const float* pb = sm + S::H2T + (16 * jt + r) * STH + 4 * q;
#pragma unroll
        for (int js = 0; js < NJS; ++js) { ao[js] = lds128(pa + 16 * js); bh[js] = lds128(pb + 16 * js); }
        HFENCE();
        f32x4 acc[2] = {f32x4{0.f, 0.f, 0.f, 0.f}, f32x4{0.f, 0.f, 0.f, 0.f}};
#pragma unroll
        for (int js = 0; js < NJS; ++js)
#pragma unroll
          for (int e = 0; e < 4; ++e) acc[js] = MFMA_F32(ao[js][e], bh[js][e], acc[js]);
#pragma unroll
        for (int i = 0; i < 4; ++i) gWhr[i] += acc[0][i] + acc[1][i];
        float s = ((ao[0][0] + ao[0][1]) + (ao[0][2] + ao[0][3])) + ((ao[1][0] + ao[1][1]) + (ao[1][2] + ao[1][3]));
        s = quad_rows_sum(s);
        const float sl = sm[S::PLS + r] + sm[S::PLS + 16 + r];
        gex += w == W_BH ? s : ((!DISC && role == 0 && w == W_LS) ? sl : 0.f);
      }
      if (book) {
        mb_s0 += sm[S::PST + 0] + sm[S::PST + 8];
        mb_s1 += sm[S::PST + 1] + sm[S::PST + 9];
        mb_s2 += sm[S::PST + 2] + sm[S::PST + 10];
        mb_s3 += sm[S::PST + 3] + sm[S::PST + 11];
        if (DISC) mb_s4 += sm[S::PST + 4] + sm[S::PST + 12];
      }
      if (!last_chunk) lds_barrier();
      STAMP(3)
    }

#if ICRL_HALVES_NORM_LOOK_EARLY
    u64 v_early = 0;
#endif
    {
      f32x4 gsc = f32x4{gb1r, gb2r, gex, 0.f};
      if (!ICRL_HALVES_EARLY_PUBLISH) {
        raw_store_u(xmine + 1 * THH * 16, gW2r[0]);
        raw_store_u(xmine + 2 * THH * 16, gW2r[1]);
      }
      raw_store_u(xmine + 0 * THH * 16, gW1r);
      if (lowk) {
        raw_store_u(xmine + 3 * THH * 16, gWhr);
        raw_store_u(xmine + 4 * THH * 16, gsc);
      }
      if (book) {
        raw_store_u(xmine + 5 * THH * 16, f32x4{mb_s0, mb_s1, mb_s2, mb_s3});
        if (DISC) raw_store_u(xmine + 6 * THH * 16, f32x4{mb_s4, 0.f, 0.f, 0.f});
      }
      asm volatile("s_waitcnt vmcnt(0)" ::: "memory");
      if (lane == 0) {
        if (xcd_local) __builtin_amdgcn_raw_buffer_store_b32(step, grs, xmine + HX_FLAG + 64 * w, 0, 1);
        else __builtin_amdgcn_raw_buffer_store_b32(step, grs, xmine + HX_FLAG + 64 * w, 0, 16);
      }
#if ICRL_HALVES_ADAM_PRE
      {
        const float omw1_ = 1.f - w1;
#pragma unroll
        for (int i = 0; i < 4; ++i) { mW1[i] *= omw1_; vW1[i] *= adam_b2f; mW2[0][i] *= omw1_; vW2[0][i] *= adam_b2f; mW2[1][i] *= omw1_; vW2[1][i] *= adam_b2f; }
        if (lowk) {
#pragma unroll
          for (int i = 0; i < 4; ++i) { mWh[i] *= omw1_; vWh[i] *= adam_b2f; }
          mb1 *= omw1_; vb1 *= adam_b2f; mb2 *= omw1_; vb2 *= adam_b2f; mex *= omw1_; vex *= adam_b2f;
        }
      }
#endif
#if ICRL_HALVES_FIRST_LOOK
      unsigned fl_a = 0, fl_b = 0, fl_c = 0;
      if (NQ == 4 && owner) {
        const int fo = xrole + HX_FLAG + 64 * w;
        fl_a = __builtin_amdgcn_raw_buffer_load_b32(grs, fo + ((half + 1) & 3) * HX_BLK, 0, 16);
        fl_b = __builtin_amdgcn_raw_buffer_load_b32(grs, fo + ((half + 2) & 3) * HX_BLK, 0, 16);
        fl_c = __builtin_amdgcn_raw_buffer_load_b32(grs, fo + ((half + 3) & 3) * HX_BLK, 0, 16);
      }
#endif
      if (STAGE_HOP) {
        commit_rows(xcur == S::XT0 ? S::XT1 : S::XT0);
        stats_partials(__builtin_amdgcn_readfirstlane(ps_next.z) & NB_MASK);
      }
      bool timed_out = false;
#if ICRL_HALVES_NORM_LOOK_EARLY
      if (NQ == 4 && tid < 24 && (tid >> 3) != role) v_early = __hip_atomic_load(nx + (step & 1) * 32 + tid, __ATOMIC_RELAXED, __HIP_MEMORY_SCOPE_AGENT);
#endif
      if constexpr (NQ == 4) {
#if ICRL_HALVES_FLAGS_TOGETHER
        if (owner) {
          const int fo = xrole + HX_FLAG + 64 * w;
          const int ka = (half + 1) & 3, kb = (half + 2) & 3, kc = (half + 3) & 3;
          int spins = 0;
#if ICRL_HALVES_FIRST_LOOK
          const bool first_ok = fl_a == step && fl_b == step && fl_c == step;
#else
          const bool first_ok = false;
#endif
          while (!first_ok) {
            const unsigned fa = __builtin_amdgcn_raw_buffer_load_b32(grs, fo + ka * HX_BLK, 0, 16);
            const unsigned fb = __builtin_amdgcn_raw_buffer_load_b32(grs, fo + kb * HX_BLK, 0, 16);
            const unsigned fc = __builtin_amdgcn_raw_buffer_load_b32(grs, fo + kc * HX_BLK, 0, 16);
            if (((fa ^ step) | (fb ^ step) | (fc ^ step)) == 0u) break;
            if (++spins >= (1 << 22)) { timed_out = true; break; }
            __builtin_amdgcn_s_sleep(1);
          }
          asm volatile("" ::: "memory");
        }
        auto wait_flag = [&](int) {};
#else
        auto wait_flag = [&](int k) {
          int spins = 0;
          while (true) {
            const unsigned f = __builtin_amdgcn_raw_buffer_load_b32(grs, xrole + k * HX_BLK + HX_FLAG + 64 * w, 0, 16);
            if (f == step) break;
            if (++spins >= (1 << 22)) { timed_out = true; break; }
            __builtin_amdgcn_s_sleep(1);
          }
          asm volatile("" ::: "memory");
        };
#endif
#if ICRL_HALVES_PARTNER_SUM && !ICRL_HALVES_OWNER_ADAM && ICRL_HALVES_FLAGS_TOGETHER
        {
          (void)wait_flag;
          const int xa = xrole + (half ^ 1) * HX_BLK, xb = xrole + (half ^ 2) * HX_BLK, xc = xrole + (half ^ 3) * HX_BLK;
          const f32x4 a0 = raw_load_u(xa + 0 * THH * 16), b0 = raw_load_u(xb + 0 * THH * 16), c0 = raw_load_u(xc + 0 * THH * 16);
          const f32x4 a1 = raw_load_u(xa + 1 * THH * 16), b1 = raw_load_u(xb + 1 * THH * 16), c1 = raw_load_u(xc + 1 * THH * 16);
          const f32x4 a2 = raw_load_u(xa + 2 * THH * 16), b2 = raw_load_u(xb + 2 * THH * 16), c2 = raw_load_u(xc + 2 * THH * 16);
#pragma unroll
          for (int i = 0; i < 4; ++i) {
            gW1r[i] = (gW1r[i] + a0[i]) + (b0[i] + c0[i]);
            gW2r[0][i] = (gW2r[0][i] + a1[i]) + (b1[i] + c1[i]);
            gW2r[1][i] = (gW2r[1][i] + a2[i]) + (b2[i] + c2[i]);
          }
          if (lowk) {
            const f32x4 a3 = raw_load_u(xa + 3 * THH * 16), b3 = raw_load_u(xb + 3 * THH * 16), c3 = raw_load_u(xc + 3 * THH * 16);
            const f32x4 a4 = raw_load_u(xa + 4 * THH * 16), b4 = raw_load_u(xb + 4 * THH * 16), c4 = raw_load_u(xc + 4 * THH * 16);
#pragma unroll
            for (int i = 0; i < 4; ++i) {
              gWhr[i] = (gWhr[i] + a3[i]) + (b3[i] + c3[i]);
              gsc[i] = (gsc[i] + a4[i]) + (b4[i] + c4[i]);
            }
            gb1r = gsc[0]; gb2r = gsc[1]; gex = gsc[2];
          }
          if (w == 7) {
            const f32x4 a5 = raw_load_u(xa + 5 * THH * 16), b5 = raw_load_u(xb + 5 * THH * 16), c5 = raw_load_u(xc + 5 * THH * 16);
            mb_s0 = (mb_s0 + a5[0]) + (b5[0] + c5[0]); mb_s1 = (mb_s1 + a5[1]) + (b5[1] + c5[1]);
            mb_s2 = (mb_s2 + a5[2]) + (b5[2] + c5[2]); mb_s3 = (mb_s3 + a5[3]) + (b5[3] + c5[3]);
            if (DISC) {
              const f32x4 a6 = raw_load_u(xa + 6 * THH * 16), b6 = raw_load_u(xb + 6 * THH * 16), c6 = raw_load_u(xc + 6 * THH * 16);
              mb_s4 = (mb_s4 + a6[0]) + (b6[0] + c6[0]);
            }
          }
        }
#else
        struct Part { f32x4 g0, g1, g2, g3, g4, b0, b1; };
        const f32x4 z4 = f32x4{0.f, 0.f, 0.f, 0.f};
        const Part own = {gW1r, gW2r[0], gW2r[1], gWhr, gsc, f32x4{mb_s0, mb_s1, mb_s2, mb_s3}, f32x4{mb_s4, 0.f, 0.f, 0.f}};
        auto fetch = [&](int k) -> Part {
          if (k == half) return own;
          wait_flag(k);
          const int xb = xrole + k * HX_BLK;
          Part p = {raw_load(xb + (0 * THH + tid) * 16), raw_load(xb + (1 * THH + tid) * 16), raw_load(xb + (2 * THH + tid) * 16), z4, z4, z4, z4};
          if (lowk) { p.g3 = raw_load(xb + (3 * THH + tid) * 16); p.g4 = raw_load(xb + (4 * THH + tid) * 16); }
          if (book) { p.b0 = raw_load(xb + (5 * THH + tid) * 16); if (DISC) p.b1 = raw_load(xb + (6 * THH + tid) * 16); }
          return p;
        };
        auto add = [&](const Part& x, const Part& y) -> Part {
          Part r;
#pragma unroll
          for (int i = 0; i < 4; ++i) {
            r.g0[i] = x.g0[i] + y.g0[i]; r.g1[i] = x.g1[i] + y.g1[i]; r.g2[i] = x.g2[i] + y.g2[i]; r.g3[i] = x.g3[i] + y.g3[i];
            r.g4[i] = x.g4[i] + y.g4[i]; r.b0[i] = x.b0[i] + y.b0[i]; r.b1[i] = x.b1[i] + y.b1[i];
          }
          return r;
        };
        if (owner) {
          const Part s01 = add(fetch(0), fetch(1));
          const Part s23 = add(fetch(2), fetch(3));
          const Part t = add(s01, s23);
          gW1r = t.g0; gW2r[0] = t.g1; gW2r[1] = t.g2; gWhr = t.g3; gsc = t.g4;
          gb1r = gsc[0]; gb2r = gsc[1]; gex = gsc[2];
          mb_s0 = t.b0[0]; mb_s1 = t.b0[1]; mb_s2 = t.b0[2]; mb_s3 = t.b0[3]; mb_s4 = t.b1[0];
        }
#endif
      } else {
#if ICRL_HALVES_POLL_ROLL
      unsigned pq0, pq1, pq2, pq3;
#endif
      {
        int spins = 0;
#if ICRL_HALVES_POLL_ROLL
        typedef int rsrc4 __attribute__((ext_vector_type(4)));
        const unsigned long long gbase = (unsigned long long)gxp;
        rsrc4 rs4;
        rs4[0] = __builtin_amdgcn_readfirstlane((int)(unsigned)gbase);
        rs4[1] = __builtin_amdgcn_readfirstlane((int)(unsigned)((gbase >> 32) & 0xffffu));
        rs4[2] = (int)ICRL_PPO_SPLIT_BYTES;
        rs4[3] = 0x00020000;
        const int foff = xtheirs + HX_FLAG + 64 * w;
        int left = 1 << 20;
        asm volatile(
            "buffer_load_dword %0, %5, %6, 0 offen sc1\n\t"
            "s_sleep 2\n\t"
            "buffer_load_dword %1, %5, %6, 0 offen sc1\n\t"
            "s_sleep 2\n\t"
            "buffer_load_dword %2, %5, %6, 0 offen sc1\n\t"
            "s_sleep 2\n\t"
            "buffer_load_dword %3, %5, %6, 0 offen sc1\n\t"
            "1:\n\t"
            "s_waitcnt vmcnt(3)\n\t"
            "v_cmp_eq_u32_e32 vcc, %7, %0\n\t"
            "s_cbranch_vccnz 2f\n\t"
            "buffer_load_dword %0, %5, %6, 0 offen sc1\n\t"
            "s_waitcnt vmcnt(3)\n\t"
            "v_cmp_eq_u32_e32 vcc, %7, %1\n\t"
            "s_cbranch_vccnz 2f\n\t"
            "buffer_load_dword %1, %5, %6, 0 offen sc1\n\t"
            "s_waitcnt vmcnt(3)\n\t"
            "v_cmp_eq_u32_e32 vcc, %7, %2\n\t"
            "s_cbranch_vccnz 2f\n\t"
            "buffer_load_dword %2, %5, %6, 0 offen sc1\n\t"
            "s_waitcnt vmcnt(3)\n\t"
            "v_cmp_eq_u32_e32 vcc, %7, %3\n\t"
            "s_cbranch_vccnz 2f\n\t"
            "buffer_load_dword %3, %5, %6, 0 offen sc1\n\t"
            "s_sub_i32 %4, %4, 1\n\t"
            "s_cmp_gt_i32 %4, 0\n\t"
            "s_cbranch_scc1 1b\n\t"
            "2:\n\t"
            : "=&v"(pq0), "=&v"(pq1), "=&v"(pq2), "=&v"(pq3), "+s"(left)
            : "v"(foff), "s"(rs4), "s"(step)
            : "vcc", "scc", "memory");
        timed_out = left <= 0;
        (void)spins;
#else
        while (true) {
          const unsigned f = __builtin_amdgcn_raw_buffer_load_b32(grs, xtheirs + HX_FLAG + 64 * w, 0, 16);
          if (f == step) break;
          if (++spins >= (1 << 22)) { timed_out = true; break; }
          __builtin_amdgcn_s_sleep(1);
        }
#endif
      }
      asm volatile("" ::: "memory");
      const f32x4 c0 = raw_load(xtheirs + (0 * THH + tid) * 16), c1 = raw_load(xtheirs + (1 * THH + tid) * 16), c2 = raw_load(xtheirs + (2 * THH + tid) * 16);
      f32x4 c3 = f32x4{0.f, 0.f, 0.f, 0.f}, c4 = c3, c5 = c3, c6 = c3;
      if (lowk) { c3 = raw_load(xtheirs + (3 * THH + tid) * 16); c4 = raw_load(xtheirs + (4 * THH + tid) * 16); }
      if (book) { c5 = raw_load(xtheirs + (5 * THH + tid) * 16); if (DISC) c6 = raw_load(xtheirs + (6 * THH + tid) * 16); }
#pragma unroll
      for (int i = 0; i < 4; ++i) { gW1r[i] += c0[i]; gW2r[0][i] += c1[i]; gW2r[1][i] += c2[i]; gWhr[i] += c3[i]; gsc[i] += c4[i]; }
#if ICRL_HALVES_POLL_ROLL
      asm volatile("" :: "v"(pq0), "v"(pq1), "v"(pq2), "v"(pq3), "v"(gW2r[1][3]));
#endif
      gb1r = gsc[0]; gb2r = gsc[1]; gex = gsc[2];
      mb_s0 += c5[0]; mb_s1 += c5[1]; mb_s2 += c5[2]; mb_s3 += c5[3]; mb_s4 += c6[0];
      }
      if (timed_out) sm[S::MISC + 13] = 1.f;
    }

    if (!DISC && role == 0 && w == W_LS && ro < A) gex += -ent_coef;

    float ss = 0.f;
#pragma unroll
    for (int i = 0; i < 4; ++i) ss = fmaf(gW1r[i], gW1r[i], ss);
#pragma unroll
    for (int cc = 0; cc < 2; ++cc)
#pragma unroll
      for (int i = 0; i < 4; ++i) ss = fmaf(gW2r[cc][i], gW2r[cc][i], ss);
    {
      float sb = 0.f;
      if (lowk) {
#pragma unroll
        for (int i = 0; i < 4; ++i) ss = fmaf(gWhr[i], gWhr[i], ss);
        sb = ex_g >= 0 ? gex * gex : 0.f;
        sb = fmaf(gb1r, gb1r, gb2r * gb2r) + sb;
      }
      ss += q == 0 ? sb : 0.f;
    }
    ss = wave_sum_fast(ss);
    if (lane == 0 && owner) {
      bool want_stop = false;
      float mean_kl = 0.f;
      const bool last_mb = (ps.nb_flags >> NB_LAST) & 1;
      const int epoch = ps.nb_flags >> NB_EPOCH;
      if (book && role == 0) {
        if ((ps.nb_flags >> NB_FIRST) & 1) *acc_kl = 0.f;
        lds_add(acc_kl, mb_s3 * inv_nb);
        if (last_mb) {
          mean_kl = __hip_atomic_load(acc_kl, __ATOMIC_RELAXED, __HIP_MEMORY_SCOPE_WORKGROUP) * inv_n_mb;
          const TrainArgs* k_ = KARGS();
          if (k_->hp.use_target_kl && mean_kl > 1.5f * k_->hp.target_kl) { want_stop = true; early_stop_epoch = epoch; }
        }
      }
      const unsigned tag = step | (want_stop ? 0x80000000u : 0u);
      if (xcd_local) __hip_atomic_store(nx + (step & 1) * 32 + role * 8 + w, ((u64)tag << 32) | (u64)__float_as_uint(ss), __ATOMIC_RELAXED, __HIP_MEMORY_SCOPE_WORKGROUP);
      else __hip_atomic_store(nx + (step & 1) * 32 + role * 8 + w, ((u64)tag << 32) | (u64)__float_as_uint(ss), __ATOMIC_RELAXED, __HIP_MEMORY_SCOPE_AGENT);
      if (!OWNER) {
        sm[S::MISC + 24 + role * 8 + w] = ss;
        if (book && role == 0) sm[S::MISC + 12] = want_stop ? 1.f : 0.f;
      }
      if (book) {
        ++steps_done;
        if (role == 0) {
          float ent = 0.f;
          if (DISC) ent = mb_s4 * inv_nb;
          else ent = sm[S::MISC + 22];
          const float entropy_loss = -ent;
          const float pl = (-(mb_s0 * inv_nb) + nu * (mb_s1 * inv_nb)) * __builtin_amdgcn_rcpf(1.f + nu);
          lds_add(acc_ent, entropy_loss); lds_add(acc_pg, pl); lds_add(acc_cf, mb_s2 * inv_nb);
          *acc_last = pl + ent_coef * entropy_loss;
          if (last_mb && (OWNER || half == 0)) { float* stats = KARGS()->stats; stats[32 + epoch] = mean_kl; stats[7] = mean_kl; }
        } else {
          const float vl = mb_s0 * inv_nb;
          lds_add(acc_vl, vl);
          *acc_last = vl;
        }
      }
    }
    STAMP(4)
    constexpr bool APRE = ICRL_HALVES_ADAM_PRELOAD && !OWNER;
    f32x4 ap_w1 = f32x4{0.f, 0.f, 0.f, 0.f}, ap_w2a = ap_w1, ap_w2b = ap_w1, ap_wh = ap_w1, ap_b = ap_w1;
    if (APRE) {
      ap_w1 = load_own_w1(); ap_w2a = load_own_w2(0); ap_w2b = load_own_w2(1);
      if (lowk) { ap_wh = load_own_wh(); ap_b = f32x4{sm[S::B1 + jb], sm[S::B2 + jb], sm[ex_s], 0.f}; }
    }
    const int xnext = xcur == S::XT0 ? S::XT1 : S::XT0;
    const int nb_next = __builtin_amdgcn_readfirstlane(ps_next.z) & NB_MASK;
    const int ptid = tid - 64 * ((NQ == 4 && !ICRL_HALVES_NORM_LOOK_EARLY) ? ICRL_HALVES_POLL_WAVE : 0);
    const bool poller = ptid >= 0 && ptid < 24 && (OWNER || (ptid >> 3) != role);
    const u64* const slot = nx + (step & 1) * 32 + ((ptid >= 0 && ptid < 24) ? ptid : 0);
#if ICRL_HALVES_EARLY_POLL
    u64 v_first = 0;
#if ICRL_HALVES_NORM_LOOK_EARLY
    if (NQ == 4 && !OWNER) v_first = v_early;
    if (poller && (unsigned)((v_first >> 32) & 0x7fffffffu) != step) v_first = __hip_atomic_load(slot, __ATOMIC_RELAXED, __HIP_MEMORY_SCOPE_AGENT);
#else
    if (poller) v_first = __hip_atomic_load(slot, __ATOMIC_RELAXED, __HIP_MEMORY_SCOPE_AGENT);
#endif
#endif
    if (!STAGE_HOP) {
      commit_rows(xnext);
      stats_partials(nb_next);
    }
    xcur = xnext;
    if (poller) {
      u64 v = 0;
      int spins = 0;
      bool ok = false;
#if ICRL_HALVES_EARLY_POLL
      v = v_first;
      ok = (unsigned)((v >> 32) & 0x7fffffffu) == step;
#endif
      while (!ok && spins < (1 << 24)) {
        v = __hip_atomic_load(slot, __ATOMIC_RELAXED, __HIP_MEMORY_SCOPE_AGENT);
        if ((unsigned)((v >> 32) & 0x7fffffffu) == step) { ok = true; break; }
        __builtin_amdgcn_s_sleep(1);
        ++spins;
      }
      sm[S::MISC + 24 + ptid] = __uint_as_float((unsigned)(v & 0xffffffffu));
      if (ptid == 7) sm[S::MISC + 12] = (v >> 63) ? 1.f : 0.f;
      if (!ok) sm[S::MISC + 13] = 1.f;
    }
    lds_barrier();
    STAMP(5)
    if (deep_pf) {
      const int idx_now = idx_next;
      idx_next = idx_nx2;
      idx_nx2 = chunk_idx(pc_nx3);
      pc_nx3 = ld_chunk(g_chunk + 4);
      issue_rows(idx_now);
    }
    float total = 0.f;
    {
#pragma unroll
      for (int g = 0; g < 6; ++g) {
        const f32x4 n = lds128(sm + S::MISC + 24 + 4 * g);
        total += (n[0] + n[1]) + (n[2] + n[3]);
      }
      const f32x4 fl = lds128(sm + S::MISC + 12);
      stop = fl[0] != 0.f;
      if (fl[1] != 0.f) { status = 1; stop = true; }
    }
    total = __builtin_amdgcn_sqrtf(total);
    float coef = max_grad_norm * __builtin_amdgcn_rcpf(total + 1e-6f);
    coef = coef > 1.f ? 1.f : coef;
    read_stats(nb_next > 0 ? nb_next : 2);

    {
      const float step_size = ps.step_size, inv_bc2_sqrt = ps.inv_bc2_sqrt;
      const float epsf = adam_epsf;
      const float omw1 = 1.f - w1, b2f_ = adam_b2f;
      const float cw1 = coef * w1, c2w2 = (coef * coef) * w2;
      auto adamn = [&](auto NE, const f32x4& g, f32x4& m, f32x4& v, f32x4& p) {
        constexpr int E = decltype(NE)::value;
        f32x4 d = f32x4{1.f, 1.f, 1.f, 1.f};
#pragma unroll
        for (int i = 0; i < E; ++i) {
          m[i] = fmaf(cw1, g[i], ICRL_HALVES_ADAM_PRE ? m[i] : omw1 * m[i]);
          v[i] = fmaf(c2w2, g[i] * g[i], ICRL_HALVES_ADAM_PRE ? v[i] : b2f_ * v[i]);
        }
#pragma unroll
        for (int i = 0; i < E; ++i) d[i] = fmaf(__builtin_amdgcn_sqrtf(v[i]), inv_bc2_sqrt, epsf);
#pragma unroll
        for (int i = 0; i < E; ++i) p[i] = fmaf(-step_size, m[i] * __builtin_amdgcn_rcpf(d[i]), p[i]);
      };
      auto adam4 = [&](const f32x4& g, f32x4& m, f32x4& v, f32x4& p) { adamn(std::integral_constant<int, 4>{}, g, m, v, p); };
      if constexpr (OWNER) {
        const int h3 = H3_BASE + (((int)(step & 1) * 3 + role) * 4 + (w >> 1)) * H3_BLK;
        f32x4 pW1, pW2a, pW2b, pWh = f32x4{0.f, 0.f, 0.f, 0.f}, pB = pWh;
        if (owner) {
          pW1 = load_own_w1(); adam4(gW1r, mW1, vW1, pW1);
          pW2a = load_own_w2(0); adam4(gW2r[0], mW2[0], vW2[0], pW2a);
          pW2b = load_own_w2(1); adam4(gW2r[1], mW2[1], vW2[1], pW2b);
          raw_store(h3 + (0 * THH + tid) * 16, pW1); raw_store(h3 + (1 * THH + tid) * 16, pW2a); raw_store(h3 + (2 * THH + tid) * 16, pW2b);
          if (lowk) {
            f32x4 g_ = f32x4{gb1r, gb2r, ex_g >= 0 ? gex : 0.f, 0.f}, m_ = f32x4{mb1, mb2, mex, 0.f}, v_ = f32x4{vb1, vb2, vex, 0.f};
            pB = f32x4{sm[S::B1 + jb], sm[S::B2 + jb], sm[ex_s], 0.f};
            adam4(g_, m_, v_, pB);
            mb1 = m_[0]; mb2 = m_[1]; mex = m_[2]; vb1 = v_[0]; vb2 = v_[1]; vex = v_[2];
            pWh = load_own_wh(); adam4(gWhr, mWh, vWh, pWh);
            raw_store(h3 + (3 * THH + tid) * 16, pWh); raw_store(h3 + (4 * THH + tid) * 16, pB);
          }
          asm volatile("s_waitcnt vmcnt(0)" ::: "memory");
          if (lane == 0) {
            if (xcd_local) __builtin_amdgcn_raw_buffer_store_b32(step, grs, h3 + H3_FLAG + 64 * w, 0, 1);
            else __builtin_amdgcn_raw_buffer_store_b32(step, grs, h3 + H3_FLAG + 64 * w, 0, 16);
          }
        } else {
          int spins = 0;
          while (true) {
            const unsigned f = __builtin_amdgcn_raw_buffer_load_b32(grs, h3 + H3_FLAG + 64 * w, 0, 16);
            if (f == step) break;
            if (++spins >= (1 << 22)) { sm[S::MISC + 13] = 1.f; status = 1; break; }
            __builtin_amdgcn_s_sleep(1);
          }
          asm volatile("" ::: "memory");
          pW1 = raw_load(h3 + (0 * THH + tid) * 16); pW2a = raw_load(h3 + (1 * THH + tid) * 16); pW2b = raw_load(h3 + (2 * THH + tid) * 16);
          if (lowk) { pWh = raw_load(h3 + (3 * THH + tid) * 16); pB = raw_load(h3 + (4 * THH + tid) * 16); }
        }
        store_w1(pW1); store_w2(0, pW2a); store_w2(1, pW2b);
        if (lowk) {
          if (q == 0) { sm[S::B1 + jb] = pB[0]; sm[S::B2 + jb] = pB[1]; sm[ex_s] = pB[2]; }
          store_wh(pWh);
          __builtin_amdgcn_s_waitcnt(0xC07F);
          refresh_gauss();
        }
      } else {
      { f32x4 p_ = APRE ? ap_w1 : load_own_w1(); adam4(gW1r, mW1, vW1, p_); store_w1(p_); }
      if (lowk) {
        f32x4 g_ = f32x4{gb1r, gb2r, ex_g >= 0 ? gex : 0.f, 0.f}, p_ = APRE ? ap_b : f32x4{sm[S::B1 + jb], sm[S::B2 + jb], sm[ex_s], 0.f};
        f32x4 m_ = f32x4{mb1, mb2, mex, 0.f}, v_ = f32x4{vb1, vb2, vex, 0.f};
        const bool has_ex = w == W_BH || (!DISC && role == 0 && w == W_LS);
        if (!ICRL_HALVES_ADAM_TRIM) adam4(g_, m_, v_, p_);
        else if (has_ex) adamn(std::integral_constant<int, 3>{}, g_, m_, v_, p_);
        else adamn(std::integral_constant<int, 2>{}, g_, m_, v_, p_);
        mb1 = m_[0]; mb2 = m_[1]; mex = m_[2]; vb1 = v_[0]; vb2 = v_[1]; vex = v_[2];
        if (q == 0) { sm[S::B1 + jb] = p_[0]; sm[S::B2 + jb] = p_[1]; sm[ex_s] = p_[2]; }
      }
#pragma unroll
      for (int cc = 0; cc < 2; ++cc) { f32x4 p_ = APRE ? (cc == 0 ? ap_w2a : ap_w2b) : load_own_w2(cc); adam4(gW2r[cc], mW2[cc], vW2[cc], p_); store_w2(cc, p_); }
      if (lowk) {
        {
          f32x4 p_ = APRE ? ap_wh : load_own_wh();
          const int ngw = (n_out + 3) >> 2;
          if (!ICRL_HALVES_ADAM_TRIM || ngw > 2) adam4(gWhr, mWh, vWh, p_);
          else if (ngw == 2) adamn(std::integral_constant<int, 2>{}, gWhr, mWh, vWh, p_);
          else adamn(std::integral_constant<int, 1>{}, gWhr, mWh, vWh, p_);
          store_wh(p_);
        }
        __builtin_amdgcn_s_waitcnt(0xC07F);
        refresh_gauss();
      }
      }
    }
    lds_barrier();
    STAMP(6)
  }

  __syncthreads();
  if (OWNER ? owner : half == 0) {
  const TrainArgs* kw = ka;
  asm volatile("" : "+s"(kw));
  const TrainArgs& a = *kw;
  const PolLayout& L = a.L;
  const int gW1 = L.W1[role], gb1 = L.b1[role], gW2 = L.W2[role], gb2 = L.b2[role];
  const int gWh = role == 0 ? L.Wa : (role == 1 ? L.Wv : L.Wc);
  {
    const f32x4 pv = load_own_w1();
#pragma unroll
    for (int i = 0; i < 4; ++i) {
      const int j = 16 * jt + 4 * q + i, k = 16 * kh + r;
      if (k < O) { a.params[gW1 + j * O + k] = pv[i]; a.exp_avg[gW1 + j * O + k] = mW1[i]; a.exp_avg_sq[gW1 + j * O + k] = vW1[i]; }
    }
  }
#pragma unroll
  for (int cc = 0; cc < 2; ++cc) {
    const f32x4 pv = load_own_w2(cc);
#pragma unroll
    for (int i = 0; i < 4; ++i) {
      const int j = 16 * jt + 4 * q + i, k = 16 * (2 * kh + cc) + r;
      a.params[gW2 + j * HD + k] = pv[i];
      a.exp_avg[gW2 + j * HD + k] = mW2[cc][i];
      a.exp_avg_sq[gW2 + j * HD + k] = vW2[cc][i];
    }
  }
  if (lowk) {
    const f32x4 pv = load_own_wh();
#pragma unroll
    for (int i = 0; i < 4; ++i) {
      const int o = out_of(i), j = 16 * jt + r;
      if (o < n_out) { a.params[gWh + o * HD + j] = pv[i]; a.exp_avg[gWh + o * HD + j] = mWh[i]; a.exp_avg_sq[gWh + o * HD + j] = vWh[i]; }
    }
    if (q == 0 && ex_g >= 0) { a.params[ex_g] = sm[ex_s]; a.exp_avg[ex_g] = mex; a.exp_avg_sq[ex_g] = vex; }
    if (q == 0) {
      a.params[gb1 + jb] = sm[S::B1 + jb]; a.exp_avg[gb1 + jb] = mb1; a.exp_avg_sq[gb1 + jb] = vb1;
      a.params[gb2 + jb] = sm[S::B2 + jb]; a.exp_avg[gb2 + jb] = mb2; a.exp_avg_sq[gb2 + jb] = vb2;
    }
  }
  if (tid == 0 && prof) {
    for (int k = 0; k < 7; ++k) {
      const int slot = 12 + 7 * role + k;
      if (slot < 32) a.stats[slot] = (float)((double)ph[k] / (double)(a.n_steps > 0 ? a.n_steps : 1));
    }
  }
  if (book) {
    if (role == 0) {
      a.stats[0] = (float)early_stop_epoch;
      a.stats[1] = (float)steps_done;
      a.stats[2] = *acc_ent; a.stats[3] = *acc_pg; a.stats[6] = *acc_cf;
      a.stats[8] = *acc_last;
      a.stats[11] = (float)status;
      a.adam_t[0] = t0 + steps_done;
    } else if (role == 1) {
      a.stats[4] = *acc_vl; a.stats[9] = *acc_last;
    } else {
      a.stats[5] = *acc_vl; a.stats[10] = *acc_last;
    }
  }
  }
}

template <int NT1, bool DISC, int OBS, int NQ, bool PROF>
__global__ void __launch_bounds__(THH) ppo_train_halves_kernel(TrainArgs a, int packed) {
  int run = 0, j = (int)blockIdx.x;
  if (packed && !packed_slot(3 * NQ, 1, run, j)) return;
  const TrainArgs* const ka = (const TrainArgs*)__builtin_amdgcn_kernarg_segment_ptr();
  if constexpr (ICRL_HALVES_ROLE_SPEC && OBS == 18 && NQ == 4 && !DISC) {
    const int role = j % 3;
    if (role == 0) ppo_train_halves_body<NT1, DISC, OBS, false, NQ, 0, PROF>(a, ka, j);
    else if (role == 1) ppo_train_halves_body<NT1, DISC, OBS, false, NQ, 1, PROF>(a, ka, j);
    else ppo_train_halves_body<NT1, DISC, OBS, false, NQ, 2, PROF>(a, ka, j);
  } else {
    ppo_train_halves_body<NT1, DISC, OBS, false, NQ, -1, PROF>(a, ka, j);
  }
}

template <int NT1, bool DISC, int OBS, int NQ, bool PROF>
__global__ void __launch_bounds__(THH) ppo_train_halves_batch_kernel(const TrainArgs* __restrict__ runs, int n_runs, int packed) {
  int run = (int)blockIdx.y, j = (int)blockIdx.x;
  if (packed && !packed_slot(3 * NQ, n_runs, run, j)) return;
  const TrainArgs* const ka = as_global(runs + run);
  ppo_train_halves_body<NT1, DISC, OBS, true, NQ, -1, PROF>(*ka, ka, j);
}

template <int NT1, bool DISC, int OBS, int NQ, bool PROF>
static int launch_halves(const TrainArgs* one, const TrainArgs* d_args, int n_runs, hipStream_t s) {
  static_assert(SmemH<NT1>::TOTAL * sizeof(float) <= 160 * 1024, "LDS budget");
  if (one != nullptr) {
    TrainArgs arg = *one;
    return launch_update_single(ppo_train_halves_kernel<NT1, DISC, OBS, NQ, PROF>, 3 * NQ, dim3(THH), 0, s, arg);
  }
  const int pg = packed_grid(3 * NQ, n_runs);
  hipLaunchKernelGGL((ppo_train_halves_batch_kernel<NT1, DISC, OBS, NQ, PROF>), pg ? dim3(pg) : dim3(3 * NQ, n_runs), dim3(THH), 0, s, d_args, n_runs, pg ? 1 : 0);
  return (int)hipGetLastError();
}

template <int NQ, bool PROF>
static int dispatch_halves_p(const TrainArgs* one, const TrainArgs* d_args, int n_runs, int obs, bool discrete, hipStream_t s) {
  if (!discrete && obs == 18) return launch_halves<2, false, 18, NQ, PROF>(one, d_args, n_runs, s);
  if (discrete && obs == 1) return launch_halves<2, true, 1, NQ, PROF>(one, d_args, n_runs, s);
  return discrete ? launch_halves<2, true, 0, NQ, PROF>(one, d_args, n_runs, s) : launch_halves<2, false, 0, NQ, PROF>(one, d_args, n_runs, s);
}
template <int NQ>
static int dispatch_halves(const TrainArgs* one, const TrainArgs* d_args, int n_runs, int obs, bool discrete, bool prof, hipStream_t s) {
  return prof ? dispatch_halves_p<NQ, true>(one, d_args, n_runs, obs, discrete, s) : dispatch_halves_p<NQ, false>(one, d_args, n_runs, obs, discrete, s);
}

int launch_train_halves(const TrainArgs& a, bool discrete, int parts, hipStream_t s) {
  const bool prof = (a.hp._pad & 1) != 0;
  return parts == 4 ? dispatch_halves<4>(&a, nullptr, 1, a.L.O, discrete, prof, s) : dispatch_halves<2>(&a, nullptr, 1, a.L.O, discrete, prof, s);
}
int launch_train_halves_batch(const TrainArgs* d_args, int n_runs, int obs, bool discrete, int parts, bool prof, hipStream_t s) {
  return parts == 4 ? dispatch_halves<4>(nullptr, d_args, n_runs, obs, discrete, prof, s) : dispatch_halves<2>(nullptr, d_args, n_runs, obs, discrete, prof, s);
}

}
```

Baseline: 937,400.

## Replace flag-based four-part gradient exchange with self-validating sentinel-tagged payloads

```diff
diff --git a/icrl_amd/csrc/ppo_common.h b/icrl_amd/csrc/ppo_common.h
--- a/icrl_amd/csrc/ppo_common.h
+++ b/icrl_amd/csrc/ppo_common.h
@@ -131,8 +131,10 @@
 
 int launch_train_rows(const TrainArgs& a, int nt1, bool discrete, bool split, hipStream_t s);
 int launch_train_pairs(const TrainArgs& a, int nt1, bool discrete, hipStream_t s);
-int launch_train_halves(const TrainArgs& a, bool discrete, int parts, hipStream_t s);
-int launch_train_halves_batch(const TrainArgs* d_args, int n_runs, int obs, bool discrete, int parts, bool prof, hipStream_t s);
+int launch_train_halves(const TrainArgs& a, bool discrete, int parts, bool tagged, hipStream_t s);
+int launch_train_halves_batch(const TrainArgs* d_args, int n_runs, int obs, bool discrete, int parts, bool prof, bool tagged, hipStream_t s);
+constexpr unsigned HALVES_EMPTY = 0x7FA5C3E1u;
+constexpr int HALVES_TAG_BYTES = 3 * 3 * 4 * (7 * 512 * 16 + 8 * 64);
 int launch_train_quarters_wide(const TrainArgs& a, bool discrete, hipStream_t s);
 int launch_train_quarters_wide2(const TrainArgs& a, bool discrete, hipStream_t s);
 constexpr int HALVES_MAX_RUNS = 40;
diff --git a/icrl_amd/csrc/ppo_train.hip b/icrl_amd/csrc/ppo_train.hip
--- a/icrl_amd/csrc/ppo_train.hip
+++ b/icrl_amd/csrc/ppo_train.hip
@@ -1,3 +1,5 @@
+#include <string.h>
+
 #include "ppo_common.h"
 
 namespace icrl {
@@ -848,6 +850,11 @@
 static bool quarters_default() {
   static const int v = [] { const char* e = getenv("ICRL_QUARTERS"); return e != nullptr ? (e[0] == '1' ? 1 : 0) : 1; }();
   return v != 0;
+}
+
+static bool halves_tagged_default() {
+  static const bool v = [] { const char* e = getenv("ICRL_HALVES_XCHG"); return e == nullptr || strcmp(e, "flags") != 0; }();
+  return v;
 }
 
 static int prepare_train(const icrl_policy_t* pol, float* exp_avg, float* exp_avg_sq, int32_t* adam_step, const icrl_buffer_t* buf,
@@ -908,7 +915,12 @@
   if (split || halves || quarters_wide) {
     const size_t off = (ICRL_PPO_PLAN_BYTES(n_steps) + 4 * (size_t)hp->n_epochs * n_total + 255) / 256 * 256;
     a.gx = reinterpret_cast<u64*>((char*)sync_ws + off);
-    e = hipMemsetAsync(a.gx, 0, ICRL_PPO_SPLIT_BYTES, s);
+    const size_t tag_bytes = quarters && halves_tagged_default() ? (size_t)HALVES_TAG_BYTES : 0;
+    if (tag_bytes) {
+      e = hipMemsetD32Async((hipDeviceptr_t)a.gx, (int)HALVES_EMPTY, tag_bytes / 4, s);
+      if (e != hipSuccess) return bad((int)e);
+    }
+    e = hipMemsetAsync((char*)a.gx + tag_bytes, 0, ICRL_PPO_SPLIT_BYTES - tag_bytes, s);
     if (e != hipSuccess) return bad((int)e);
   }
   if (quarters_wide) return quarters_wide2 ? 7 : 6;
@@ -954,7 +966,7 @@
   const int kind = prepare_train(pol, exp_avg, exp_avg_sq, adam_step, buf, perms, nu, hp, stats, sync_ws, s, a, &err, 1);
   if (kind < 0) return err;
   const int nt1 = (pol->obs_dim + 15) / 16;
-  if (kind == 4 || kind == 5) return launch_train_halves(a, pol->discrete != 0, kind == 5 ? 4 : 2, s);
+  if (kind == 4 || kind == 5) return launch_train_halves(a, pol->discrete != 0, kind == 5 ? 4 : 2, kind == 5 && halves_tagged_default(), s);
   if (kind == 6) return launch_train_quarters_wide(a, pol->discrete != 0, s);
   if (kind == 7) return launch_train_quarters_wide2(a, pol->discrete != 0, s);
   if (kind == 0) return launch_train_pairs(a, nt1, pol->discrete != 0, s);
@@ -998,7 +1010,7 @@
     if (e != 0) return e;
   }
   const int nt1 = (j0.pol->obs_dim + 15) / 16;
-  if (kind0 == 4 || kind0 == 5) return launch_train_halves_batch(d_args, n_runs, j0.pol->obs_dim, j0.pol->discrete != 0, kind0 == 5 ? 4 : 2, (j0.hp->_pad & 1) != 0, s);
+  if (kind0 == 4 || kind0 == 5) return launch_train_halves_batch(d_args, n_runs, j0.pol->obs_dim, j0.pol->discrete != 0, kind0 == 5 ? 4 : 2, (j0.hp->_pad & 1) != 0, kind0 == 5 && halves_tagged_default(), s);
   if (kind0 == 0) return launch_train_pairs_batch(d_args, n_runs, j0.pol->obs_dim, nt1, j0.pol->discrete != 0, (j0.hp->_pad & 1) != 0, s);
   return launch_train_rows_batch(d_args, n_runs, nt1, j0.pol->discrete != 0, kind0 == 2, s);
 }
diff --git a/icrl_amd/csrc/ppo_train_halves.hip b/icrl_amd/csrc/ppo_train_halves.hip
--- a/icrl_amd/csrc/ppo_train_halves.hip
+++ b/icrl_amd/csrc/ppo_train_halves.hip
@@ -22,12 +22,6 @@
 #endif
 #ifndef ICRL_HALVES_POLL_ROLL
 #define ICRL_HALVES_POLL_ROLL 0
-#endif
-#ifndef ICRL_HALVES_OWNER_ADAM
-#define ICRL_HALVES_OWNER_ADAM 0
-#endif
-#ifndef ICRL_HALVES_FLAGS_TOGETHER
-#define ICRL_HALVES_FLAGS_TOGETHER 1
 #endif
 #ifndef ICRL_HALVES_PARTNER_SUM
 #define ICRL_HALVES_PARTNER_SUM 1
@@ -68,9 +62,6 @@
 #endif
 #ifndef ICRL_HALVES_POLL_WAVE
 #define ICRL_HALVES_POLL_WAVE 4
-#endif
-#ifndef ICRL_HALVES_FIRST_LOOK
-#define ICRL_HALVES_FIRST_LOOK 0
 #endif
 #ifndef ICRL_HALVES_NORM_LOOK_EARLY
 #define ICRL_HALVES_NORM_LOOK_EARLY 0
@@ -89,10 +80,8 @@
 constexpr int HX_GROUPS = 7;
 constexpr int HX_FLAG = HX_GROUPS * THH * 16;
 constexpr int HX_BLK = HX_FLAG + 8 * 64;
-constexpr int H3_FLAG = 5 * THH * 16;
-constexpr int H3_BLK = H3_FLAG + 8 * 64;
-constexpr int H3_BASE = 24 * HX_BLK;
-static_assert(H3_BASE + 24 * H3_BLK + 3 * 512 <= (int)ICRL_PPO_SPLIT_BYTES, "the exchange of up to four row parts per network lives in the split workspace");
+static_assert(HALVES_TAG_BYTES == 3 * 3 * 4 * HX_BLK, "ppo_common.h: the area the launcher fills with HALVES_EMPTY");
+static_assert(HALVES_TAG_BYTES + 3 * 512 <= (int)ICRL_PPO_SPLIT_BYTES, "the exchange of up to four row parts per network lives in the split workspace");
 
 template <int NT1>
 struct SmemH {
@@ -168,7 +157,7 @@
   return sm;
 }
 
-template <int NT1, bool DISC, int OBS, bool BATCH, int NQ, int ROLE_T = -1, bool PROF = false>
+template <int NT1, bool DISC, int OBS, bool BATCH, int NQ, int ROLE_T = -1, bool PROF = false, bool TAG = false>
 __device__ __forceinline__ void ppo_train_halves_body(const TrainArgs& a, const TrainArgs* const ka, const int slot_j) {
 #define GPH(x) (BATCH ? as_global(x) : (x))
   using S = SmemH<NT1>;
@@ -176,6 +165,7 @@
   static_assert(NT1 == 2, "one observation tile per weight-gradient wave half");
   float* const sm = halves_smem<NT1>();
   static_assert(NQ == 2 || NQ == 4, "two or four row parts per network");
+  static_assert(!TAG || NQ == 4, "the self-validating exchange is the four-part form's");
   constexpr int HRQ = RB / NQ;
   constexpr int NJS = HRQ / 16;
   if ((a.hp._pad & 64) && slot_j == 3 * NQ - 1) return;
@@ -188,8 +178,6 @@
   const int rt2 = SPREAD ? w >> 2 : w & 1, fq = SPREAD ? w & 3 : w >> 1;
   const int qp0 = SPREAD ? w ^ 1 : w ^ 2, qp1 = SPREAD ? w ^ 2 : w ^ 4, qp2 = SPREAD ? w ^ 3 : w ^ 6;
   const bool fwd_wave = rt2 < NJS;
-  constexpr bool OWNER = NQ == 4 && ICRL_HALVES_OWNER_ADAM;
-  const bool owner = !OWNER || (w >> 1) == half;
   constexpr bool STAGE_HOP = ICRL_HALVES_STAGE_IN_HOP || NQ == 4;
   const int jt = w & 3, kh = w >> 2;
   const int r = lane & 15, q = lane >> 4;
@@ -303,7 +291,7 @@
   const float max_grad_norm = a.hp.max_grad_norm, adam_epsf = a.hp.adam_eps, adam_b2f = a.hp.adam_beta2;
   u64* const xch0 = GPH(a.xch);
   u64* const gxp = GPH(a.gx);
-  u64* const nx = (half == 0 || OWNER) ? xch0 : reinterpret_cast<u64*>(reinterpret_cast<char*>(gxp) + ICRL_PPO_SPLIT_BYTES - 512 * half);
+  u64* const nx = half == 0 ? xch0 : reinterpret_cast<u64*>(reinterpret_cast<char*>(gxp) + ICRL_PPO_SPLIT_BYTES - 512 * half);
 
   constexpr bool STAGE_IDLE = ICRL_HALVES_STAGE_IDLE && NQ == 4;
   const int gb_row = STAGE_IDLE ? (tid >> 4) & 15 : tid >> 4, gpart = tid & 15;
@@ -489,7 +477,8 @@
     issue_stats(sidx_next);
     sidx_next = stat_idx(ps_nx2);
     float mb_s0 = 0.f, mb_s1 = 0.f, mb_s2 = 0.f, mb_s3 = 0.f, mb_s4 = 0.f;
-    const int xrole = ((int)(step & 1) * 3 + role) * NQ * HX_BLK;
+    const int xbuf = TAG ? (int)(step % 3u) : (int)(step & 1);
+    const int xrole = (xbuf * 3 + role) * NQ * HX_BLK;
     const int xmine = xrole + half * HX_BLK, xtheirs = xrole + (1 - half) * HX_BLK;
 
     const int n_chunks = (nb + RB - 1) / RB;
@@ -842,23 +831,33 @@
 #endif
     {
       f32x4 gsc = f32x4{gb1r, gb2r, gex, 0.f};
+      if constexpr (TAG) __builtin_amdgcn_s_waitcnt(0x0F70);
+      auto xstore = [&](int uni_off, f32x4 v) {
+        if constexpr (TAG) {
+#pragma unroll
+          for (int i = 0; i < 4; ++i) v[i] = __builtin_canonicalizef(v[i]);
+        }
+        raw_store_u(uni_off, v);
+      };
       if (!ICRL_HALVES_EARLY_PUBLISH) {
-        raw_store_u(xmine + 1 * THH * 16, gW2r[0]);
-        raw_store_u(xmine + 2 * THH * 16, gW2r[1]);
-      }
-      raw_store_u(xmine + 0 * THH * 16, gW1r);
+        xstore(xmine + 1 * THH * 16, gW2r[0]);
+        xstore(xmine + 2 * THH * 16, gW2r[1]);
+      }
+      xstore(xmine + 0 * THH * 16, gW1r);
       if (lowk) {
-        raw_store_u(xmine + 3 * THH * 16, gWhr);
-        raw_store_u(xmine + 4 * THH * 16, gsc);
-      }
-      if (book) {
-        raw_store_u(xmine + 5 * THH * 16, f32x4{mb_s0, mb_s1, mb_s2, mb_s3});
-        if (DISC) raw_store_u(xmine + 6 * THH * 16, f32x4{mb_s4, 0.f, 0.f, 0.f});
-      }
-      asm volatile("s_waitcnt vmcnt(0)" ::: "memory");
-      if (lane == 0) {
-        if (xcd_local) __builtin_amdgcn_raw_buffer_store_b32(step, grs, xmine + HX_FLAG + 64 * w, 0, 1);
-        else __builtin_amdgcn_raw_buffer_store_b32(step, grs, xmine + HX_FLAG + 64 * w, 0, 16);
+        xstore(xmine + 3 * THH * 16, gWhr);
+        xstore(xmine + 4 * THH * 16, gsc);
+      }
+      if (TAG ? w == 7 : book) {
+        xstore(xmine + 5 * THH * 16, f32x4{mb_s0, mb_s1, mb_s2, mb_s3});
+        if (DISC) xstore(xmine + 6 * THH * 16, f32x4{mb_s4, 0.f, 0.f, 0.f});
+      }
+      if constexpr (!TAG) {
+        asm volatile("s_waitcnt vmcnt(0)" ::: "memory");
+        if (lane == 0) {
+          if (xcd_local) __builtin_amdgcn_raw_buffer_store_b32(step, grs, xmine + HX_FLAG + 64 * w, 0, 1);
+          else __builtin_amdgcn_raw_buffer_store_b32(step, grs, xmine + HX_FLAG + 64 * w, 0, 16);
+        }
       }
 #if ICRL_HALVES_ADAM_PRE
       {
@@ -872,15 +871,6 @@
         }
       }
 #endif
-#if ICRL_HALVES_FIRST_LOOK
-      unsigned fl_a = 0, fl_b = 0, fl_c = 0;
-      if (NQ == 4 && owner) {
-        const int fo = xrole + HX_FLAG + 64 * w;
-        fl_a = __builtin_amdgcn_raw_buffer_load_b32(grs, fo + ((half + 1) & 3) * HX_BLK, 0, 16);
-        fl_b = __builtin_amdgcn_raw_buffer_load_b32(grs, fo + ((half + 2) & 3) * HX_BLK, 0, 16);
-        fl_c = __builtin_amdgcn_raw_buffer_load_b32(grs, fo + ((half + 3) & 3) * HX_BLK, 0, 16);
-      }
-#endif
       if (STAGE_HOP) {
         commit_rows(xcur == S::XT0 ? S::XT1 : S::XT0);
         stats_partials(__builtin_amdgcn_readfirstlane(ps_next.z) & NB_MASK);
@@ -889,18 +879,77 @@
 #if ICRL_HALVES_NORM_LOOK_EARLY
       if (NQ == 4 && tid < 24 && (tid >> 3) != role) v_early = __hip_atomic_load(nx + (step & 1) * 32 + tid, __ATOMIC_RELAXED, __HIP_MEMORY_SCOPE_AGENT);
 #endif
-      if constexpr (NQ == 4) {
-#if ICRL_HALVES_FLAGS_TOGETHER
-        if (owner) {
+      if constexpr (NQ == 4 && TAG) {
+        const int xpeer[3] = {xrole + (half ^ 1) * HX_BLK, xrole + (half ^ 2) * HX_BLK, xrole + (half ^ 3) * HX_BLK};
+        const bool has3 = lowk || w == 7, has4 = lowk || (DISC && w == 7);
+        const int goff[5] = {0, 1 * THH * 16, 2 * THH * 16, (lowk ? 3 : 5) * THH * 16, (lowk ? 4 : 6) * THH * 16};
+        const f32x4 z4 = f32x4{0.f, 0.f, 0.f, 0.f};
+        f32x4 x3 = lowk ? gWhr : f32x4{mb_s0, mb_s1, mb_s2, mb_s3}, x4 = lowk ? gsc : f32x4{mb_s4, 0.f, 0.f, 0.f};
+        auto fetch3 = [&](int g, f32x4 (&p)[3]) {
+#pragma unroll
+          for (int k = 0; k < 3; ++k) p[k] = raw_load_u(xpeer[k] + goff[g]);
+        };
+        auto sum3 = [&](f32x4& o, const f32x4 (&p)[3]) -> bool {
+#pragma unroll
+          for (int i = 0; i < 4; ++i) o[i] = (o[i] + p[0][i]) + (p[1][i] + p[2][i]);
+          return __builtin_isunordered(o[0], o[1]) | __builtin_isunordered(o[2], o[3]);
+        };
+        {
+          f32x4 p0[3], p1[3], p2[3], p3[3] = {z4, z4, z4}, p4[3] = {z4, z4, z4};
+          fetch3(0, p0); fetch3(1, p1); fetch3(2, p2);
+          if (has3) fetch3(3, p3);
+          if (has4) fetch3(4, p4);
+          bool bad = sum3(gW1r, p0);
+          bad |= sum3(gW2r[0], p1);
+          bad |= sum3(gW2r[1], p2);
+          bad |= sum3(x3, p3);
+          bad |= sum3(x4, p4);
+          if (__builtin_expect(__builtin_amdgcn_ballot_w64(bad) != 0ull, 0)) {
+            asm volatile("s_waitcnt vmcnt(0)" ::: "memory");
+            f32x4 pg[5][3], own[5] = {z4, z4, z4, z4, z4};
+#pragma unroll
+            for (int k = 0; k < 3; ++k) { pg[3][k] = z4; pg[4][k] = z4; }
+            const unsigned all = 0x7u * (1u | 8u | 64u | (has3 ? 512u : 0u) | (has4 ? 4096u : 0u));
+            unsigned miss = all;
+            for (int spins = 0;; ++spins) {
+#pragma unroll
+              for (int g = 0; g < 5; ++g)
+#pragma unroll
+                for (int k = 0; k < 3; ++k)
+                  if (miss & (1u << (3 * g + k))) pg[g][k] = raw_load_u(xpeer[k] + goff[g]);
+              miss = 0;
+#pragma unroll
+              for (int g = 0; g < 5; ++g)
+#pragma unroll
+                for (int k = 0; k < 3; ++k) {
+                  const raw_u4 u = __builtin_bit_cast(raw_u4, pg[g][k]);
+                  const bool e = u[0] == HALVES_EMPTY || u[1] == HALVES_EMPTY || u[2] == HALVES_EMPTY || u[3] == HALVES_EMPTY;
+                  if (__builtin_amdgcn_ballot_w64(e) != 0ull) miss |= 1u << (3 * g + k);
+                }
+              if (miss == 0u) break;
+              if (spins >= (1 << 22)) { timed_out = true; break; }
+              __builtin_amdgcn_s_sleep(2);
+            }
+#pragma unroll
+            for (int g = 0; g < 5; ++g)
+              if (all & (1u << (3 * g))) own[g] = raw_load_u(xmine + goff[g]);
+#pragma unroll
+            for (int g = 0; g < 5; ++g) (void)sum3(own[g], pg[g]);
+            gW1r = own[0]; gW2r[0] = own[1]; gW2r[1] = own[2]; x3 = own[3]; x4 = own[4];
+          }
+        }
+        if (lowk) {
+          gWhr = x3; gsc = x4;
+          gb1r = gsc[0]; gb2r = gsc[1]; gex = gsc[2];
+        } else {
+          mb_s0 = x3[0]; mb_s1 = x3[1]; mb_s2 = x3[2]; mb_s3 = x3[3]; mb_s4 = x4[0];
+        }
+      } else if constexpr (NQ == 4) {
+        {
           const int fo = xrole + HX_FLAG + 64 * w;
           const int ka = (half + 1) & 3, kb = (half + 2) & 3, kc = (half + 3) & 3;
           int spins = 0;
-#if ICRL_HALVES_FIRST_LOOK
-          const bool first_ok = fl_a == step && fl_b == step && fl_c == step;
-#else
-          const bool first_ok = false;
-#endif
-          while (!first_ok) {
+          while (true) {
             const unsigned fa = __builtin_amdgcn_raw_buffer_load_b32(grs, fo + ka * HX_BLK, 0, 16);
             const unsigned fb = __builtin_amdgcn_raw_buffer_load_b32(grs, fo + kb * HX_BLK, 0, 16);
             const unsigned fc = __builtin_amdgcn_raw_buffer_load_b32(grs, fo + kc * HX_BLK, 0, 16);
@@ -910,22 +959,8 @@
           }
           asm volatile("" ::: "memory");
         }
-        auto wait_flag = [&](int) {};
-#else
-        auto wait_flag = [&](int k) {
-          int spins = 0;
-          while (true) {
-            const unsigned f = __builtin_amdgcn_raw_buffer_load_b32(grs, xrole + k * HX_BLK + HX_FLAG + 64 * w, 0, 16);
-            if (f == step) break;
-            if (++spins >= (1 << 22)) { timed_out = true; break; }
-            __builtin_amdgcn_s_sleep(1);
-          }
-          asm volatile("" ::: "memory");
-        };
-#endif
-#if ICRL_HALVES_PARTNER_SUM && !ICRL_HALVES_OWNER_ADAM && ICRL_HALVES_FLAGS_TOGETHER
+#if ICRL_HALVES_PARTNER_SUM
         {
-          (void)wait_flag;
           const int xa = xrole + (half ^ 1) * HX_BLK, xb = xrole + (half ^ 2) * HX_BLK, xc = xrole + (half ^ 3) * HX_BLK;
           const f32x4 a0 = raw_load_u(xa + 0 * THH * 16), b0 = raw_load_u(xb + 0 * THH * 16), c0 = raw_load_u(xc + 0 * THH * 16);
           const f32x4 a1 = raw_load_u(xa + 1 * THH * 16), b1 = raw_load_u(xb + 1 * THH * 16), c1 = raw_load_u(xc + 1 * THH * 16);
@@ -962,7 +997,6 @@
         const Part own = {gW1r, gW2r[0], gW2r[1], gWhr, gsc, f32x4{mb_s0, mb_s1, mb_s2, mb_s3}, f32x4{mb_s4, 0.f, 0.f, 0.f}};
         auto fetch = [&](int k) -> Part {
           if (k == half) return own;
-          wait_flag(k);
           const int xb = xrole + k * HX_BLK;
           Part p = {raw_load(xb + (0 * THH + tid) * 16), raw_load(xb + (1 * THH + tid) * 16), raw_load(xb + (2 * THH + tid) * 16), z4, z4, z4, z4};
           if (lowk) { p.g3 = raw_load(xb + (3 * THH + tid) * 16); p.g4 = raw_load(xb + (4 * THH + tid) * 16); }
@@ -978,7 +1012,7 @@
           }
           return r;
         };
-        if (owner) {
+        {
           const Part s01 = add(fetch(0), fetch(1));
           const Part s23 = add(fetch(2), fetch(3));
           const Part t = add(s01, s23);
@@ -1082,7 +1116,7 @@
       ss += q == 0 ? sb : 0.f;
     }
     ss = wave_sum_fast(ss);
-    if (lane == 0 && owner) {
+    if (lane == 0) {
       bool want_stop = false;
       float mean_kl = 0.f;
       const bool last_mb = (ps.nb_flags >> NB_LAST) & 1;
@@ -1099,10 +1133,8 @@
       const unsigned tag = step | (want_stop ? 0x80000000u : 0u);
       if (xcd_local) __hip_atomic_store(nx + (step & 1) * 32 + role * 8 + w, ((u64)tag << 32) | (u64)__float_as_uint(ss), __ATOMIC_RELAXED, __HIP_MEMORY_SCOPE_WORKGROUP);
       else __hip_atomic_store(nx + (step & 1) * 32 + role * 8 + w, ((u64)tag << 32) | (u64)__float_as_uint(ss), __ATOMIC_RELAXED, __HIP_MEMORY_SCOPE_AGENT);
-      if (!OWNER) {
-        sm[S::MISC + 24 + role * 8 + w] = ss;
-        if (book && role == 0) sm[S::MISC + 12] = want_stop ? 1.f : 0.f;
-      }
+      sm[S::MISC + 24 + role * 8 + w] = ss;
+      if (book && role == 0) sm[S::MISC + 12] = want_stop ? 1.f : 0.f;
       if (book) {
         ++steps_done;
         if (role == 0) {
@@ -1113,7 +1145,7 @@
           const float pl = (-(mb_s0 * inv_nb) + nu * (mb_s1 * inv_nb)) * __builtin_amdgcn_rcpf(1.f + nu);
           lds_add(acc_ent, entropy_loss); lds_add(acc_pg, pl); lds_add(acc_cf, mb_s2 * inv_nb);
           *acc_last = pl + ent_coef * entropy_loss;
-          if (last_mb && (OWNER || half == 0)) { float* stats = KARGS()->stats; stats[32 + epoch] = mean_kl; stats[7] = mean_kl; }
+          if (last_mb && half == 0) { float* stats = KARGS()->stats; stats[32 + epoch] = mean_kl; stats[7] = mean_kl; }
         } else {
           const float vl = mb_s0 * inv_nb;
           lds_add(acc_vl, vl);
@@ -1122,7 +1154,7 @@
       }
     }
     STAMP(4)
-    constexpr bool APRE = ICRL_HALVES_ADAM_PRELOAD && !OWNER;
+    constexpr bool APRE = ICRL_HALVES_ADAM_PRELOAD;
     f32x4 ap_w1 = f32x4{0.f, 0.f, 0.f, 0.f}, ap_w2a = ap_w1, ap_w2b = ap_w1, ap_wh = ap_w1, ap_b = ap_w1;
     if (APRE) {
       ap_w1 = load_own_w1(); ap_w2a = load_own_w2(0); ap_w2b = load_own_w2(1);
@@ -1131,12 +1163,12 @@
     const int xnext = xcur == S::XT0 ? S::XT1 : S::XT0;
     const int nb_next = __builtin_amdgcn_readfirstlane(ps_next.z) & NB_MASK;
     const int ptid = tid - 64 * ((NQ == 4 && !ICRL_HALVES_NORM_LOOK_EARLY) ? ICRL_HALVES_POLL_WAVE : 0);
-    const bool poller = ptid >= 0 && ptid < 24 && (OWNER || (ptid >> 3) != role);
+    const bool poller = ptid >= 0 && ptid < 24 && (ptid >> 3) != role;
     const u64* const slot = nx + (step & 1) * 32 + ((ptid >= 0 && ptid < 24) ? ptid : 0);
 #if ICRL_HALVES_EARLY_POLL
     u64 v_first = 0;
 #if ICRL_HALVES_NORM_LOOK_EARLY
-    if (NQ == 4 && !OWNER) v_first = v_early;
+    if (NQ == 4) v_first = v_early;
     if (poller && (unsigned)((v_first >> 32) & 0x7fffffffu) != step) v_first = __hip_atomic_load(slot, __ATOMIC_RELAXED, __HIP_MEMORY_SCOPE_AGENT);
 #else
     if (poller) v_first = __hip_atomic_load(slot, __ATOMIC_RELAXED, __HIP_MEMORY_SCOPE_AGENT);
@@ -1165,6 +1197,21 @@
       if (ptid == 7) sm[S::MISC + 12] = (v >> 63) ? 1.f : 0.f;
       if (!ok) sm[S::MISC + 13] = 1.f;
     }
+    if constexpr (TAG) {
+      const int xold = ((xbuf == 0 ? 2 : xbuf - 1) * 3 + role) * NQ * HX_BLK + half * HX_BLK;
+      const f32x4 e4 = __builtin_bit_cast(f32x4, raw_u4{HALVES_EMPTY, HALVES_EMPTY, HALVES_EMPTY, HALVES_EMPTY});
+      raw_store_u(xold + 0 * THH * 16, e4);
+      raw_store_u(xold + 1 * THH * 16, e4);
+      raw_store_u(xold + 2 * THH * 16, e4);
+      if (lowk) {
+        raw_store_u(xold + 3 * THH * 16, e4);
+        raw_store_u(xold + 4 * THH * 16, e4);
+      }
+      if (w == 7) {
+        raw_store_u(xold + 5 * THH * 16, e4);
+        if (DISC) raw_store_u(xold + 6 * THH * 16, e4);
+      }
+    }
     lds_barrier();
     STAMP(5)
     if (deep_pf) {
@@ -1209,47 +1256,6 @@
         for (int i = 0; i < E; ++i) p[i] = fmaf(-step_size, m[i] * __builtin_amdgcn_rcpf(d[i]), p[i]);
       };
       auto adam4 = [&](const f32x4& g, f32x4& m, f32x4& v, f32x4& p) { adamn(std::integral_constant<int, 4>{}, g, m, v, p); };
-      if constexpr (OWNER) {
-        const int h3 = H3_BASE + (((int)(step & 1) * 3 + role) * 4 + (w >> 1)) * H3_BLK;
-        f32x4 pW1, pW2a, pW2b, pWh = f32x4{0.f, 0.f, 0.f, 0.f}, pB = pWh;
-        if (owner) {
-          pW1 = load_own_w1(); adam4(gW1r, mW1, vW1, pW1);
-          pW2a = load_own_w2(0); adam4(gW2r[0], mW2[0], vW2[0], pW2a);
-          pW2b = load_own_w2(1); adam4(gW2r[1], mW2[1], vW2[1], pW2b);
-          raw_store(h3 + (0 * THH + tid) * 16, pW1); raw_store(h3 + (1 * THH + tid) * 16, pW2a); raw_store(h3 + (2 * THH + tid) * 16, pW2b);
-          if (lowk) {
-            f32x4 g_ = f32x4{gb1r, gb2r, ex_g >= 0 ? gex : 0.f, 0.f}, m_ = f32x4{mb1, mb2, mex, 0.f}, v_ = f32x4{vb1, vb2, vex, 0.f};
-            pB = f32x4{sm[S::B1 + jb], sm[S::B2 + jb], sm[ex_s], 0.f};
-            adam4(g_, m_, v_, pB);
-            mb1 = m_[0]; mb2 = m_[1]; mex = m_[2]; vb1 = v_[0]; vb2 = v_[1]; vex = v_[2];
-            pWh = load_own_wh(); adam4(gWhr, mWh, vWh, pWh);
-            raw_store(h3 + (3 * THH + tid) * 16, pWh); raw_store(h3 + (4 * THH + tid) * 16, pB);
-          }
-          asm volatile("s_waitcnt vmcnt(0)" ::: "memory");
-          if (lane == 0) {
-            if (xcd_local) __builtin_amdgcn_raw_buffer_store_b32(step, grs, h3 + H3_FLAG + 64 * w, 0, 1);
-            else __builtin_amdgcn_raw_buffer_store_b32(step, grs, h3 + H3_FLAG + 64 * w, 0, 16);
-          }
-        } else {
-          int spins = 0;
-          while (true) {
-            const unsigned f = __builtin_amdgcn_raw_buffer_load_b32(grs, h3 + H3_FLAG + 64 * w, 0, 16);
-            if (f == step) break;
-            if (++spins >= (1 << 22)) { sm[S::MISC + 13] = 1.f; status = 1; break; }
-            __builtin_amdgcn_s_sleep(1);
-          }
-          asm volatile("" ::: "memory");
-          pW1 = raw_load(h3 + (0 * THH + tid) * 16); pW2a = raw_load(h3 + (1 * THH + tid) * 16); pW2b = raw_load(h3 + (2 * THH + tid) * 16);
-          if (lowk) { pWh = raw_load(h3 + (3 * THH + tid) * 16); pB = raw_load(h3 + (4 * THH + tid) * 16); }
-        }
-        store_w1(pW1); store_w2(0, pW2a); store_w2(1, pW2b);
-        if (lowk) {
-          if (q == 0) { sm[S::B1 + jb] = pB[0]; sm[S::B2 + jb] = pB[1]; sm[ex_s] = pB[2]; }
-          store_wh(pWh);
-          __builtin_amdgcn_s_waitcnt(0xC07F);
-          refresh_gauss();
-        }
-      } else {
       { f32x4 p_ = APRE ? ap_w1 : load_own_w1(); adam4(gW1r, mW1, vW1, p_); store_w1(p_); }
       if (lowk) {
         f32x4 g_ = f32x4{gb1r, gb2r, ex_g >= 0 ? gex : 0.f, 0.f}, p_ = APRE ? ap_b : f32x4{sm[S::B1 + jb], sm[S::B2 + jb], sm[ex_s], 0.f};
@@ -1275,14 +1281,13 @@
         __builtin_amdgcn_s_waitcnt(0xC07F);
         refresh_gauss();
       }
-      }
     }
     lds_barrier();
     STAMP(6)
   }
 
   __syncthreads();
-  if (OWNER ? owner : half == 0) {
+  if (half == 0) {
   const TrainArgs* kw = ka;
   asm volatile("" : "+s"(kw));
   const TrainArgs& a = *kw;
@@ -1344,58 +1349,65 @@
   }
 }
 
-template <int NT1, bool DISC, int OBS, int NQ, bool PROF>
+template <int NT1, bool DISC, int OBS, int NQ, bool PROF, bool TAG>
 __global__ void __launch_bounds__(THH) ppo_train_halves_kernel(TrainArgs a, int packed) {
   int run = 0, j = (int)blockIdx.x;
   if (packed && !packed_slot(3 * NQ, 1, run, j)) return;
   const TrainArgs* const ka = (const TrainArgs*)__builtin_amdgcn_kernarg_segment_ptr();
   if constexpr (ICRL_HALVES_ROLE_SPEC && OBS == 18 && NQ == 4 && !DISC) {
     const int role = j % 3;
-    if (role == 0) ppo_train_halves_body<NT1, DISC, OBS, false, NQ, 0, PROF>(a, ka, j);
-    else if (role == 1) ppo_train_halves_body<NT1, DISC, OBS, false, NQ, 1, PROF>(a, ka, j);
-    else ppo_train_halves_body<NT1, DISC, OBS, false, NQ, 2, PROF>(a, ka, j);
+    if (role == 0) ppo_train_halves_body<NT1, DISC, OBS, false, NQ, 0, PROF, TAG>(a, ka, j);
+    else if (role == 1) ppo_train_halves_body<NT1, DISC, OBS, false, NQ, 1, PROF, TAG>(a, ka, j);
+    else ppo_train_halves_body<NT1, DISC, OBS, false, NQ, 2, PROF, TAG>(a, ka, j);
   } else {
-    ppo_train_halves_body<NT1, DISC, OBS, false, NQ, -1, PROF>(a, ka, j);
+    ppo_train_halves_body<NT1, DISC, OBS, false, NQ, -1, PROF, TAG>(a, ka, j);
   }
 }
 
-template <int NT1, bool DISC, int OBS, int NQ, bool PROF>
+template <int NT1, bool DISC, int OBS, int NQ, bool PROF, bool TAG>
 __global__ void __launch_bounds__(THH) ppo_train_halves_batch_kernel(const TrainArgs* __restrict__ runs, int n_runs, int packed) {
   int run = (int)blockIdx.y, j = (int)blockIdx.x;
   if (packed && !packed_slot(3 * NQ, n_runs, run, j)) return;
   const TrainArgs* const ka = as_global(runs + run);
-  ppo_train_halves_body<NT1, DISC, OBS, true, NQ, -1, PROF>(*ka, ka, j);
+  ppo_train_halves_body<NT1, DISC, OBS, true, NQ, -1, PROF, TAG>(*ka, ka, j);
 }
 
-template <int NT1, bool DISC, int OBS, int NQ, bool PROF>
+template <int NT1, bool DISC, int OBS, int NQ, bool PROF, bool TAG>
 static int launch_halves(const TrainArgs* one, const TrainArgs* d_args, int n_runs, hipStream_t s) {
   static_assert(SmemH<NT1>::TOTAL * sizeof(float) <= 160 * 1024, "LDS budget");
   if (one != nullptr) {
     TrainArgs arg = *one;
-    return launch_update_single(ppo_train_halves_kernel<NT1, DISC, OBS, NQ, PROF>, 3 * NQ, dim3(THH), 0, s, arg);
+    return launch_update_single(ppo_train_halves_kernel<NT1, DISC, OBS, NQ, PROF, TAG>, 3 * NQ, dim3(THH), 0, s, arg);
   }
   const int pg = packed_grid(3 * NQ, n_runs);
-  hipLaunchKernelGGL((ppo_train_halves_batch_kernel<NT1, DISC, OBS, NQ, PROF>), pg ? dim3(pg) : dim3(3 * NQ, n_runs), dim3(THH), 0, s, d_args, n_runs, pg ? 1 : 0);
+  hipLaunchKernelGGL((ppo_train_halves_batch_kernel<NT1, DISC, OBS, NQ, PROF, TAG>), pg ? dim3(pg) : dim3(3 * NQ, n_runs), dim3(THH), 0, s, d_args, n_runs, pg ? 1 : 0);
   return (int)hipGetLastError();
 }
 
+template <int NQ, bool PROF, bool TAG>
+static int dispatch_halves_t(const TrainArgs* one, const TrainArgs* d_args, int n_runs, int obs, bool discrete, hipStream_t s) {
+  if (!discrete && obs == 18) return launch_halves<2, false, 18, NQ, PROF, TAG>(one, d_args, n_runs, s);
+  if (discrete && obs == 1) return launch_halves<2, true, 1, NQ, PROF, TAG>(one, d_args, n_runs, s);
+  return discrete ? launch_halves<2, true, 0, NQ, PROF, TAG>(one, d_args, n_runs, s) : launch_halves<2, false, 0, NQ, PROF, TAG>(one, d_args, n_runs, s);
+}
 template <int NQ, bool PROF>
-static int dispatch_halves_p(const TrainArgs* one, const TrainArgs* d_args, int n_runs, int obs, bool discrete, hipStream_t s) {
-  if (!discrete && obs == 18) return launch_halves<2, false, 18, NQ, PROF>(one, d_args, n_runs, s);
-  if (discrete && obs == 1) return launch_halves<2, true, 1, NQ, PROF>(one, d_args, n_runs, s);
-  return discrete ? launch_halves<2, true, 0, NQ, PROF>(one, d_args, n_runs, s) : launch_halves<2, false, 0, NQ, PROF>(one, d_args, n_runs, s);
+static int dispatch_halves_p(const TrainArgs* one, const TrainArgs* d_args, int n_runs, int obs, bool discrete, bool tagged, hipStream_t s) {
+  if constexpr (NQ == 4) {
+    if (tagged) return dispatch_halves_t<NQ, PROF, true>(one, d_args, n_runs, obs, discrete, s);
+  }
+  return dispatch_halves_t<NQ, PROF, false>(one, d_args, n_runs, obs, discrete, s);
 }
 template <int NQ>
-static int dispatch_halves(const TrainArgs* one, const TrainArgs* d_args, int n_runs, int obs, bool discrete, bool prof, hipStream_t s) {
-  return prof ? dispatch_halves_p<NQ, true>(one, d_args, n_runs, obs, discrete, s) : dispatch_halves_p<NQ, false>(one, d_args, n_runs, obs, discrete, s);
+static int dispatch_halves(const TrainArgs* one, const TrainArgs* d_args, int n_runs, int obs, bool discrete, bool prof, bool tagged, hipStream_t s) {
+  return prof ? dispatch_halves_p<NQ, true>(one, d_args, n_runs, obs, discrete, tagged, s) : dispatch_halves_p<NQ, false>(one, d_args, n_runs, obs, discrete, tagged, s);
 }
 
-int launch_train_halves(const TrainArgs& a, bool discrete, int parts, hipStream_t s) {
+int launch_train_halves(const TrainArgs& a, bool discrete, int parts, bool tagged, hipStream_t s) {
   const bool prof = (a.hp._pad & 1) != 0;
-  return parts == 4 ? dispatch_halves<4>(&a, nullptr, 1, a.L.O, discrete, prof, s) : dispatch_halves<2>(&a, nullptr, 1, a.L.O, discrete, prof, s);
+  return parts == 4 ? dispatch_halves<4>(&a, nullptr, 1, a.L.O, discrete, prof, tagged, s) : dispatch_halves<2>(&a, nullptr, 1, a.L.O, discrete, prof, false, s);
 }
-int launch_train_halves_batch(const TrainArgs* d_args, int n_runs, int obs, bool discrete, int parts, bool prof, hipStream_t s) {
-  return parts == 4 ? dispatch_halves<4>(nullptr, d_args, n_runs, obs, discrete, prof, s) : dispatch_halves<2>(nullptr, d_args, n_runs, obs, discrete, prof, s);
+int launch_train_halves_batch(const TrainArgs* d_args, int n_runs, int obs, bool discrete, int parts, bool prof, bool tagged, hipStream_t s) {
+  return parts == 4 ? dispatch_halves<4>(nullptr, d_args, n_runs, obs, discrete, prof, tagged, s) : dispatch_halves<2>(nullptr, d_args, n_runs, obs, discrete, prof, false, s);
 }
 
 }
```

Result: slower. 528,900 (-43.6%).
